# yuanwu2017/llm-d

Measured on AMD Instinct MI355X. Metric: output tok/s per decode GPU + p50 TTFT, Llama-3-70B P/D-disagg on 8×MI355X, higher is better.
Workload: dtype bf16; 1 GPU; model=Llama-3-70B, global_batch=64, seq_len=5000, isl=5000, osl=250, parallelism=dp1, block_size=64, graphs=True, kv_cache_dtype=auto, async_scheduling=True, setup_prompts_landed=63

## Files before the change

### llmd_amd/csrc/ops/bindings.cpp

```cpp
#include <torch/extension.h>
#include <c10/hip/HIPGuard.h>
#include <c10/hip/HIPStream.h>
#include <hip/hip_runtime.h>
#include <pybind11/stl.h>

#include <map>
#include <mutex>
#include <memory>
#include <vector>

extern "C" {
void llmd_rms_norm(void*, int64_t, const void*, int64_t, const void*, int, int, float, hipStream_t);
void llmd_layer_norm(void*, int64_t, void*, int64_t, void*, int64_t, const void*, const void*, int, int, float,
                     hipStream_t);
void llmd_fused_add_rms_norm(void*, int64_t, void*, int64_t, const void*, int, int, float,
                             hipStream_t);
int llmd_qk_rms_norm(void*, int64_t, const void*, const void*, int, int, int, int, float, hipStream_t);
void llmd_rope_cache(void*, int64_t, const int64_t*, const float*, int, int, int, int,
                     const int64_t*, void*, void*, int64_t, int, int, int, int, float, float, hipStream_t);
void llmd_gated_act(void*, int64_t, const void*, int64_t, int, int, int, float, float, hipStream_t);
int llmd_paged_decode(const void*, int64_t, const void*, const void*, int64_t, int, const int*, int,
                      const int*, int, int, int, int, float, int, const float*, int, int, void*,
                      int64_t, float*, float*, int, float, float, const int*, const int*, const int*,
                      const int*, int, int, int, const int*, hipStream_t);
int llmd_paged_prefill(const void*, int64_t, const void*, const void*, int64_t, int, const int*, int,
                       const int*, const int*, const int*, const int*, int, int, int, int, float,
                       int, const float*, void*, int64_t, int, float, float, hipStream_t);
int llmd_prefill_tokens_per_item(int, int, int, int, int);
void llmd_sample(const void*, int64_t, int, int, int, const float*, const int64_t*, int64_t*, float*,
                 float*, int, hipStream_t);
int llmd_sample_splits(int, int);
void llmd_topk_topp_mask(float*, int64_t, int, int, const int*, const float*, const float*,
                         hipStream_t);
void llmd_top_logprobs(const void*, int64_t, int, int, int, const int*, int, int*, float*, hipStream_t);
int llmd_top_logprobs_max();
int llmd_kvx_copy_blocks(void*, const void*, int64_t, int64_t, const int*, int, const int64_t*, int,
                         int64_t, hipStream_t);
int llmd_kvx_copy_blocks2(void*, const void*, int64_t, int64_t, const int*, int, const int64_t*, int, int64_t, int,
                          hipStream_t);
int llmd_kvx_ipc_export(const void*, void*, int64_t*);
int llmd_kvx_ipc_open(const void*, void**);
int llmd_kvx_ipc_close(void*);
int llmd_mla_attention(const void*, int64_t, const void*, int64_t, int, const int*, int, const int*,
                       const int*, int, int, float, int, int, void*, int64_t, float*, float*, int, float,
                       const int*, hipStream_t);
int llmd_mla_rope_cache(const void*, int64_t, void*, int64_t, const void*, int64_t, const void*, int64_t,
                        const int64_t*, const float*, int, int, const int64_t*, void*, int64_t, int, int, float,
                        hipStream_t);
int llmd_lora_bgmv(const void*, int64_t, const void*, const void*, int, int, int, int, const int*, float*, void*,
                   int64_t, hipStream_t);
int llmd_skinny_gemm(const void*, int64_t, const void*, int64_t, int, int, int, int, int, int, void*, int64_t,
                     float*, hipStream_t);
int llmd_dgemm_supported(int, int, int);
int llmd_mgemm(const void*, int64_t, const void*, int64_t, int, int, int, int, int, int, void*, int64_t, float*,
               int*, hipStream_t);
int llmd_mgemm_lds(int, int, int);
int llmd_mgemm_partials(const void*, int64_t, const void*, int64_t, int, int, int, int, int, int, float*, hipStream_t);
int llmd_reduce_rope_cache(const float*, int, int, void*, int64_t, const int64_t*, const float*, int, int, int, int,
                           const int64_t*, void*, void*, int64_t, int, int, int, int, float, float, hipStream_t);
int llmd_mgemm_add_rmsnorm(const void*, int64_t, const void*, int64_t, int, int, int, int, int, int, float*, void*,
                           int64_t, const void*, float, void*, int64_t, hipStream_t);
int llmd_mgemm_silu(const void*, int64_t, const void*, int64_t, int, int, int, int, int, void*, int64_t, hipStream_t);
int llmd_pgemm(const void*, int64_t, const void*, int64_t, void*, int64_t, int, int, int, int, int, void*,
               hipStream_t);
int64_t llmd_pgemm_ws_bytes(int, int, int, int, int);
int llmd_pgemm_fp8(const void*, int64_t, const float*, const void*, int64_t, const float*, void*, int64_t, int, int,
                   int, int, void*, hipStream_t);
int64_t llmd_pgemm_fp8_ws_bytes(int, int, int, int);
int llmd_mgemm_fp8(const void*, int64_t, const float*, const void*, int64_t, const float*, int, int, int, int, int,
                   int, void*, int64_t, float*, int*, hipStream_t);
int llmd_vmm_granularity(int, size_t*);
int llmd_vmm_alloc(int, size_t, int, void**, uint64_t*);
int llmd_vmm_export_fd(uint64_t, int*);
int llmd_vmm_import(const int*, int, size_t, int, void**, uint64_t*);
int llmd_vmm_free(void*, size_t, int, const uint64_t*);
int llmd_kvx_handle_size();
int llmd_kvx_dma_blocks(void*, const void*, int64_t, int64_t, const int*, int, int64_t, hipStream_t);
void llmd_moe_topk(const float*, int, int, int, int, const float*, int, int, int, float, int*, float*,
                   hipStream_t);
void llmd_moe_align(const int*, int, int, int, int*, int*, int*, int, int*, int*, hipStream_t);
int llmd_moe_gemm_tile_m();
void llmd_moe_gemm(const void*, int64_t, int, const int*, const int*, int, const void*, int64_t, int, int,
                   void*, int64_t, int, int, float, float, int, const void*, hipStream_t);
void llmd_moe_combine(const void*, int64_t, const int*, const float*, int, int, int, void*, int64_t,
                      hipStream_t);
int llmd_quant_fp8_rows(const void*, int64_t, void*, int64_t, float*, int, int, hipStream_t);
void llmd_rms_norm_quant(void*, int64_t, float*, const void*, int64_t, void*, int64_t, const void*, int, int, float,
                         hipStream_t);
void llmd_gated_act_quant(void*, int64_t, float*, const void*, int64_t, int, int, int, float, float, hipStream_t);
int llmd_quant_fp8_groups(const void*, int64_t, void*, int64_t, float*, int64_t, int, int, hipStream_t);
int llmd_quant_fp8_groups_padded(const void*, int64_t, void*, int64_t, float*, int64_t, int, int, int, const int*,
                                 hipStream_t);
void llmd_moe_gemm_fp8(const void*, int64_t, const float*, int64_t, int, const int*, const int*, int, const void*,
                       int64_t, const float*, int, int, void*, int64_t, int, int, float, float, int, const void*,
                       hipStream_t);
int llmd_moe_gemm3_fp8(const void*, int64_t, const float*, int64_t, int, const int*, const int*, int, const void*,
                       int64_t, const float*, int, int, void*, int64_t, int, int, float, float, int, const void*,
                       void*, int64_t, float*, int64_t, hipStream_t);
int llmd_moe_gemm3_tile_m();
int llmd_moe_gemm4_bf16(const void*, int64_t, int, const int*, const int*, int, const void*, int64_t, int, int, void*,
                        int64_t, int, int, float, float, int, const void*, int64_t, int, hipStream_t);
int llmd_moe_gemm8_bf16(const void*, int64_t, int, const int*, const int*, const int*, int, const void*, int64_t, int,
                        int, void*, int64_t, int, int, float, float, int, const void*, int64_t, int, hipStream_t);
int llmd_moe_gemm4_fp8(const void*, int64_t, const float*, int64_t, int, const int*, const int*, int, const void*,
                       int64_t, const float*, int, int, void*, int64_t, int, int, float, float, int, const void*,
                       int64_t, int, hipStream_t);
int llmd_moe_gemm8_fp8(const void*, int64_t, const float*, int64_t, int, const int*, const int*, const int*, int,
                       const void*, int64_t, const float*, int, int, void*, int64_t, int, int, float, float, int,
                       const void*, int64_t, int, hipStream_t);
int llmd_moe_gemm3_bf16(const void*, int64_t, int, const int*, const int*, int, const void*, int64_t, int, int, void*,
                        int64_t, int, int, float, float, int, const void*, hipStream_t);
int llmd_symm_alloc(size_t, void**);
int llmd_symm_free(void*);
int64_t llmd_symm_sig_bytes();
int llmd_symm_grid();
int llmd_symm_max_ranks();
int llmd_symm_channels();
int llmd_symm_error(const void*, uint32_t*);
int llmd_symm_clear_error(void*);
int llmd_symm_host_err(int64_t*);
int llmd_symm_all_reduce(const int64_t*, int, int, int, int, int64_t, int64_t, const void*, void*, int64_t,
                         hipStream_t);
int llmd_symm_ep_dispatch(const int64_t*, int, int, int, const int64_t*, const void*, int64_t, const int*,
                          const float*, int, int, int, int, int, int, hipStream_t);
int llmd_symm_ep_combine(const int64_t*, int, int, int, const int64_t*, const void*, int64_t, const int*, int, int,
                         int, int, int, void*, int64_t, hipStream_t);
}

namespace {

std::optional<c10::DeviceIndex> dev_of(const torch::Tensor& t) {
  if (t.is_cuda()) return t.get_device();
  return std::nullopt;
}

hipStream_t cur_stream() { return c10::hip::getCurrentHIPStream().stream(); }

#define CHECK_CUDA(x) TORCH_CHECK((x).is_cuda(), #x " must be a GPU tensor")
#define CHECK_BF16(x) TORCH_CHECK((x).scalar_type() == at::kBFloat16, #x " must be bf16")
#define CHECK_INNER(x) TORCH_CHECK((x).stride(-1) == 1, #x " inner dim must be contiguous")
#define CHECK_DT(x, t) TORCH_CHECK((x).scalar_type() == (t), #x " has wrong dtype")

void rms_norm(torch::Tensor out, torch::Tensor x, torch::Tensor w, double eps) {
  const c10::hip::OptionalHIPGuard device_guard(dev_of(out));
  CHECK_CUDA(x); CHECK_BF16(x); CHECK_BF16(out); CHECK_BF16(w);
  CHECK_INNER(x); CHECK_INNER(out);
  TORCH_CHECK(x.dim() == 2 && out.dim() == 2 && w.is_contiguous(), "rms_norm: 2-D x/out");
  const int d = x.size(1);
  TORCH_CHECK(d % 8 == 0 && w.numel() == d && out.size(1) == d && out.size(0) == x.size(0),
              "rms_norm shape");
  TORCH_CHECK(x.stride(0) % 8 == 0 && out.stride(0) % 8 == 0, "rms_norm: 16-B aligned rows");
  llmd_rms_norm(out.data_ptr(), out.stride(0), x.data_ptr(), x.stride(0), w.data_ptr(), x.size(0), d,
                (float)eps, cur_stream());
}

void qk_rms_norm(torch::Tensor qkv, torch::Tensor qw, torch::Tensor kw, int64_t Hq, int64_t Hkv, double eps) {
  const c10::hip::OptionalHIPGuard device_guard(dev_of(qkv));
  CHECK_CUDA(qkv); CHECK_BF16(qkv); CHECK_BF16(qw); CHECK_BF16(kw);
  CHECK_INNER(qkv);
  TORCH_CHECK(qkv.dim() == 2, "qk_rms_norm: qkv [T, (Hq+2Hkv)*D]");
  const int64_t D = qw.numel();
  TORCH_CHECK(kw.numel() == D && qw.is_contiguous() && kw.is_contiguous(), "qk_rms_norm: weights [D]");
  TORCH_CHECK(D == 64 || D == 128 || D == 256, "qk_rms_norm: head dim 64 / 128 / 256");
  TORCH_CHECK(qkv.size(1) >= (Hq + Hkv) * D, "qk_rms_norm: qkv narrower than (Hq + Hkv) * D");
  const int rc = llmd_qk_rms_norm(qkv.data_ptr(), qkv.stride(0), qw.data_ptr(), kw.data_ptr(), qkv.size(0),
                                  (int)Hq, (int)Hkv, (int)D, (float)eps, cur_stream());
  TORCH_CHECK(rc == 0, "qk_rms_norm: unsupported head dim");
}

void fused_add_rms_norm(torch::Tensor x, torch::Tensor residual, torch::Tensor w, double eps) {
  const c10::hip::OptionalHIPGuard device_guard(dev_of(x));
  CHECK_CUDA(x); CHECK_BF16(x); CHECK_BF16(residual); CHECK_BF16(w);
  CHECK_INNER(x); CHECK_INNER(residual);
  TORCH_CHECK(x.dim() == 2 && residual.sizes() == x.sizes(), "fused_add_rms_norm shape");
  const int d = x.size(1);
  TORCH_CHECK(d % 8 == 0 && w.numel() == d && w.is_contiguous(), "fused_add_rms_norm d");
  TORCH_CHECK(x.stride(0) % 8 == 0 && residual.stride(0) % 8 == 0, "16-B aligned rows");
  llmd_fused_add_rms_norm(x.data_ptr(), x.stride(0), residual.data_ptr(), residual.stride(0),
                          w.data_ptr(), x.size(0), d, (float)eps, cur_stream());
}

void layer_norm(torch::Tensor out, torch::Tensor x, c10::optional<torch::Tensor> residual, torch::Tensor w,
                torch::Tensor b, double eps) {
  const c10::hip::OptionalHIPGuard device_guard(dev_of(x));
  CHECK_CUDA(x); CHECK_BF16(x); CHECK_BF16(out); CHECK_BF16(w); CHECK_BF16(b);
  CHECK_INNER(x); CHECK_INNER(out);
  TORCH_CHECK(x.dim() == 2 && out.sizes() == x.sizes(), "layer_norm: 2-D x/out of one shape");
  const int d = x.size(1);
  TORCH_CHECK(d % 8 == 0 && w.numel() == d && b.numel() == d && w.is_contiguous() && b.is_contiguous(),
              "layer_norm: d % 8 == 0, contiguous w/b of d elements");
  TORCH_CHECK(x.stride(0) % 8 == 0 && out.stride(0) % 8 == 0, "layer_norm: 16-B aligned rows");
  void* rp = nullptr;
  int64_t rs = 0;
  if (residual.has_value()) {
    CHECK_BF16(*residual); CHECK_INNER(*residual);
    TORCH_CHECK(residual->sizes() == x.sizes() && residual->stride(0) % 8 == 0, "layer_norm residual shape");
    rp = residual->data_ptr();
    rs = residual->stride(0);
  }
  llmd_layer_norm(out.data_ptr(), out.stride(0), x.data_ptr(), x.stride(0), rp, rs, w.data_ptr(), b.data_ptr(),
                  x.size(0), d, (float)eps, cur_stream());
}

bool is_fp8_cache(const torch::Tensor& c) {
  TORCH_CHECK(c.is_cuda(), "cache must be a GPU tensor");
  const auto t = c.scalar_type();
  TORCH_CHECK(t == at::kBFloat16 || t == at::kFloat8_e4m3fn, "KV cache must be bf16 or float8_e4m3fn");
  return t == at::kFloat8_e4m3fn;
}

void rope_cache(torch::Tensor qkv, torch::Tensor positions, torch::Tensor cos_sin, int64_t Hq,
                int64_t Hkv, int64_t D, torch::Tensor slots, torch::Tensor k_cache,
                torch::Tensor v_cache, bool neox, double k_scale, double v_scale) {
  const c10::hip::OptionalHIPGuard device_guard(dev_of(qkv));
  CHECK_CUDA(qkv); CHECK_BF16(qkv); CHECK_INNER(qkv);
  CHECK_DT(positions, at::kLong); CHECK_DT(slots, at::kLong); CHECK_DT(cos_sin, at::kFloat);
  TORCH_CHECK(qkv.dim() == 2 && qkv.size(1) >= (Hq + 2 * Hkv) * D, "rope_cache: qkv width");
  const int T = qkv.size(0);
// ... 169 lines not shown
                "mla workspace too small");
  }
  int rc = llmd_mla_attention(q.data_ptr(), q.stride(0), cache.data_ptr(), cache.stride(0), cache.size(1),
                              block_tables.data_ptr<int>(), block_tables.stride(0), row_seq.data_ptr<int>(),
                              row_len.data_ptr<int>(), R, H, (float)scale, split_size, nsplit, out.data_ptr(),
                              out.stride(0), nsplit > 1 ? part_o.data_ptr<float>() : nullptr,
                              nsplit > 1 ? part_ml.data_ptr<float>() : nullptr, f8 ? 1 : 0, (float)kv_scale,
                              sdev, cur_stream());
  TORCH_CHECK(rc == 0, "mla_attention failed: ", rc);
}

void mla_rope_cache(torch::Tensor q, torch::Tensor q_lat, torch::Tensor kv_c, torch::Tensor k_pe,
                    torch::Tensor positions, torch::Tensor cos_sin, int64_t H, torch::Tensor slots,
                    torch::Tensor cache, double kv_scale) {
  const c10::hip::OptionalHIPGuard device_guard(dev_of(q));
  CHECK_CUDA(q); CHECK_BF16(q); CHECK_BF16(q_lat); CHECK_BF16(kv_c); CHECK_BF16(k_pe);
  const bool f8 = is_fp8_cache(cache);
  TORCH_CHECK(kv_scale > 0, "mla_rope: kv_scale must be positive");
  CHECK_INNER(q); CHECK_INNER(q_lat); CHECK_INNER(kv_c); CHECK_INNER(k_pe);
  CHECK_DT(positions, at::kLong); CHECK_DT(slots, at::kLong); CHECK_DT(cos_sin, at::kFloat);
  const int T = q.size(0);
  TORCH_CHECK(q.size(1) >= H * 192 && q_lat.size(0) >= T && q_lat.size(1) >= H * 576, "mla_rope: q widths");
  TORCH_CHECK(kv_c.size(0) >= T && kv_c.size(1) == 512 && k_pe.size(0) >= T && k_pe.size(1) == 64,
              "mla_rope: kv_c [T,512], k_pe [T,64]");
  TORCH_CHECK(kv_c.stride(0) % 8 == 0, "mla_rope: 16-B aligned kv_c rows");
  TORCH_CHECK(positions.numel() >= T && slots.numel() >= T, "mla_rope: positions/slots");
  TORCH_CHECK(cos_sin.dim() == 2 && cos_sin.size(1) == 64 && cos_sin.is_contiguous(), "mla_rope: cos_sin [P,64]");
  TORCH_CHECK(cache.dim() == 3 && cache.size(2) == 576 && cache.stride(1) == 576, "mla_rope: cache [blocks,bs,576]");
  int rc = llmd_mla_rope_cache(q.data_ptr(), q.stride(0), q_lat.data_ptr(), q_lat.stride(0), kv_c.data_ptr(),
                               kv_c.stride(0), k_pe.data_ptr(), k_pe.stride(0), positions.data_ptr<int64_t>(),
                               cos_sin.data_ptr<float>(), T, H, slots.data_ptr<int64_t>(), cache.data_ptr(),
                               cache.stride(0), cache.size(1), f8 ? 1 : 0, (float)(1.0 / kv_scale), cur_stream());
  TORCH_CHECK(rc == 0, "mla_rope_cache failed: ", rc);
}

void lora_bgmv(torch::Tensor y, torch::Tensor x, torch::Tensor A, torch::Tensor B, torch::Tensor slot,
               torch::Tensor h) {
  const c10::hip::OptionalHIPGuard device_guard(dev_of(y));
  CHECK_CUDA(x); CHECK_BF16(x); CHECK_BF16(y); CHECK_BF16(A); CHECK_BF16(B); CHECK_INNER(x); CHECK_INNER(y);
  CHECK_DT(slot, at::kInt); CHECK_DT(h, at::kFloat);
  TORCH_CHECK(A.dim() == 3 && B.dim() == 3 && A.is_contiguous() && B.is_contiguous(), "lora: A [S,R,in], B [S,out,R]");
  const int T = x.size(0), R = A.size(1), in = A.size(2), out = B.size(1);
  TORCH_CHECK(B.size(0) == A.size(0) && B.size(2) == R && R <= 128, "lora: slot/rank mismatch");
  TORCH_CHECK(x.size(1) == in && y.size(0) == T && y.size(1) == out && slot.numel() >= T, "lora: shapes");
  TORCH_CHECK(in % 8 == 0 && in <= 32768 && x.stride(0) % 8 == 0, "lora: in dim");
  TORCH_CHECK(h.numel() >= (int64_t)T * R, "lora: workspace");
  int rc = llmd_lora_bgmv(x.data_ptr(), x.stride(0), A.data_ptr(), B.data_ptr(), T, R, in, out, slot.data_ptr<int>(),
                          h.data_ptr<float>(), y.data_ptr(), y.stride(0), cur_stream());
  TORCH_CHECK(rc == 0, "lora_bgmv failed: ", rc);
}

void skinny_gemm(torch::Tensor y, torch::Tensor x, torch::Tensor w, int64_t rb, int64_t nsplit, int64_t occ,
                 torch::Tensor part) {
  const c10::hip::OptionalHIPGuard device_guard(dev_of(y));
  CHECK_CUDA(x); CHECK_BF16(x); CHECK_BF16(w); CHECK_BF16(y); CHECK_INNER(x); CHECK_INNER(w); CHECK_INNER(y);
  TORCH_CHECK(x.dim() == 2 && w.dim() == 2 && y.dim() == 2, "skinny_gemm: 2-D operands");
  const int M = x.size(0), K = x.size(1), N = w.size(0);
  TORCH_CHECK(M >= 1 && M <= 64 && w.size(1) == K && K % 256 == 0, "skinny_gemm: M <= 64, K % 256 == 0");
  TORCH_CHECK(N % 4 == 0, "skinny_gemm: N % 4 == 0");
  TORCH_CHECK(y.size(0) == M && y.size(1) == N, "skinny_gemm: output shape");
  TORCH_CHECK(x.stride(0) % 8 == 0 && w.stride(0) % 8 == 0 && y.stride(0) % 4 == 0, "skinny_gemm: row alignment");
  TORCH_CHECK(llmd_dgemm_supported(M, (int)rb, (int)occ), "skinny_gemm: no kernel for rb=", rb, " occ=", occ);
  if (nsplit > 1) {
    CHECK_DT(part, at::kFloat);
    TORCH_CHECK(part.numel() >= nsplit * (int64_t)M * N, "skinny_gemm: workspace");
  }
  int rc = llmd_skinny_gemm(x.data_ptr(), x.stride(0), w.data_ptr(), w.stride(0), M, N, K, (int)rb, (int)nsplit,
                            (int)occ, y.data_ptr(), y.stride(0), nsplit > 1 ? part.data_ptr<float>() : nullptr,
                            cur_stream());
  TORCH_CHECK(rc == 0, "skinny_gemm failed: ", rc);
}

extern "C" int llmd_mla_v2_shape(int R, int fp8);
int64_t mla_v2_shape(int64_t R, bool fp8) { return llmd_mla_v2_shape((int)R, fp8 ? 1 : 0); }

bool skinny_supported(int64_t M, int64_t rb, int64_t occ) { return llmd_dgemm_supported((int)M, (int)rb, (int)occ); }

int* mgemm_counters(const torch::Device& d, int64_t tiles) {
  static const bool on = [] {
    const char* e = getenv("LLMD_MGEMM_FIXUP");
    return e && e[0] == '1';
  }();
  if (!on || tiles > 1024) return nullptr;
  static std::mutex mu;
  static std::map<int, torch::Tensor> pools;
  static std::map<int, uint32_t> next;
  std::lock_guard<std::mutex> g(mu);
  auto& t = pools[d.index()];
  if (!t.defined()) {
    hipStreamCaptureStatus cs = hipStreamCaptureStatusNone;
    if (hipStreamIsCapturing(cur_stream(), &cs) != hipSuccess || cs != hipStreamCaptureStatusNone) return nullptr;
    t = torch::zeros({256 * 1024}, torch::dtype(torch::kInt32).device(d));
  }
  const uint32_t i = next[d.index()]++ % 256;
  return t.data_ptr<int>() + (int64_t)i * 1024;
}

void mgemm(torch::Tensor y, torch::Tensor x, torch::Tensor w, int64_t wrb, int64_t nsplit, int64_t stages,
           torch::Tensor part) {
  const c10::hip::OptionalHIPGuard device_guard(dev_of(y));
  CHECK_CUDA(x); CHECK_BF16(x); CHECK_BF16(w); CHECK_BF16(y); CHECK_INNER(x); CHECK_INNER(w); CHECK_INNER(y);
  TORCH_CHECK(x.dim() == 2 && w.dim() == 2 && y.dim() == 2, "mgemm: 2-D operands");
  const int M = x.size(0), K = x.size(1), N = w.size(0);
  TORCH_CHECK(M >= 1 && M <= 256 && w.size(1) == K && K % 64 == 0, "mgemm: M <= 256, K % 64 == 0");
  TORCH_CHECK(N % 4 == 0 && y.size(0) == M && y.size(1) == N, "mgemm: output shape / N % 4");
  TORCH_CHECK(x.stride(0) % 8 == 0 && w.stride(0) % 8 == 0 && y.stride(0) % 4 == 0, "mgemm: row alignment");
  TORCH_CHECK(llmd_mgemm_lds(M, (int)wrb, (int)stages) > 0, "mgemm: no kernel for wrb=", wrb, " stages=", stages);
  if (nsplit > 1) {
    CHECK_DT(part, at::kFloat);
    TORCH_CHECK(part.numel() >= nsplit * (int64_t)M * N, "mgemm: workspace");
  }
  int rc = llmd_mgemm(x.data_ptr(), x.stride(0), w.data_ptr(), w.stride(0), M, N, K, (int)wrb, (int)nsplit,
                      (int)stages, y.data_ptr(), y.stride(0), nsplit > 1 ? part.data_ptr<float>() : nullptr,
                      nsplit > 1 ? mgemm_counters(y.device(), (N + 64 * wrb - 1) / (64 * wrb)) : nullptr,
                      cur_stream());
  TORCH_CHECK(rc == 0, "mgemm failed: ", rc);
}

void mgemm_add_rmsnorm(torch::Tensor out, torch::Tensor x, torch::Tensor w, int64_t wrb, int64_t nsplit,
                       int64_t stages, torch::Tensor part, torch::Tensor residual, torch::Tensor gamma, double eps) {
  const c10::hip::OptionalHIPGuard device_guard(dev_of(out));
  CHECK_CUDA(x); CHECK_BF16(x); CHECK_BF16(w); CHECK_BF16(out); CHECK_BF16(residual); CHECK_BF16(gamma);
  CHECK_INNER(x); CHECK_INNER(w); CHECK_INNER(out); CHECK_INNER(residual); CHECK_DT(part, at::kFloat);
  TORCH_CHECK(x.dim() == 2 && w.dim() == 2 && out.dim() == 2 && residual.dim() == 2, "mgemm_add_rmsnorm: 2-D operands");
  const int M = x.size(0), K = x.size(1), N = w.size(0);
  TORCH_CHECK(M >= 1 && M <= 128 && w.size(1) == K && K % 64 == 0 && N % 8 == 0, "mgemm_add_rmsnorm: shapes");
  TORCH_CHECK(out.size(0) == M && out.size(1) == N && residual.size(0) == M && residual.size(1) == N &&
              gamma.numel() == N, "mgemm_add_rmsnorm: output / residual / gamma shape");
  TORCH_CHECK(nsplit > 1 && part.numel() >= nsplit * (int64_t)M * N, "mgemm_add_rmsnorm: split-K workspace");
  int rc = llmd_mgemm_add_rmsnorm(x.data_ptr(), x.stride(0), w.data_ptr(), w.stride(0), M, N, K, (int)wrb,
                                  (int)nsplit, (int)stages, part.data_ptr<float>(), residual.data_ptr(),
                                  residual.stride(0), gamma.data_ptr(), (float)eps, out.data_ptr(), out.stride(0),
                                  cur_stream());
  TORCH_CHECK(rc == 0, "mgemm_add_rmsnorm failed: ", rc);
}

void pgemm(torch::Tensor y, torch::Tensor x, torch::Tensor w, int64_t epi, int64_t variant, bool split_k) {
  const c10::hip::OptionalHIPGuard device_guard(dev_of(y));
  CHECK_CUDA(x); CHECK_BF16(x); CHECK_BF16(w); CHECK_BF16(y); CHECK_INNER(x); CHECK_INNER(w); CHECK_INNER(y);
  TORCH_CHECK(x.dim() == 2 && w.dim() == 2 && y.dim() == 2, "pgemm: 2-D operands");
  const int64_t M = x.size(0), K = x.size(1), N = w.size(0);
  TORCH_CHECK(w.size(1) == K && K % 64 == 0 && N % 256 == 0, "pgemm: N % 256 == 0, K % 64 == 0");
  TORCH_CHECK(y.size(0) == M && y.size(1) == ((epi == 1 || epi == 3) ? N / 2 : N), "pgemm: output shape");
  TORCH_CHECK(epi != 3 || (variant >= 3 && variant <= 6), "pgemm: epi 3 (SiLU on the [gate; up] weight) needs variant 3-6");
  TORCH_CHECK(x.stride(0) % 8 == 0 && w.stride(0) % 8 == 0 && y.stride(0) % 8 == 0, "pgemm: 16-B row alignment");
  torch::Tensor ws;
  const int64_t wsb = split_k ? llmd_pgemm_ws_bytes((int)M, (int)N, (int)K, (int)epi, (int)variant) : 0;
  if (wsb > 0) ws = torch::empty({wsb / 4}, x.options().dtype(torch::kFloat));
  int rc = llmd_pgemm(x.data_ptr(), x.stride(0), w.data_ptr(), w.stride(0), y.data_ptr(), y.stride(0), (int)M,
                      (int)N, (int)K, (int)epi, (int)variant, wsb > 0 ? ws.data_ptr() : nullptr, cur_stream());
  TORCH_CHECK(rc == 0, "pgemm failed: ", rc);
}

void pgemm_fp8(torch::Tensor y, torch::Tensor xq, torch::Tensor xs, torch::Tensor wq, torch::Tensor ws, int64_t epi,
               bool split_k) {
  const c10::hip::OptionalHIPGuard device_guard(dev_of(y));
  CHECK_CUDA(xq); CHECK_BF16(y); CHECK_INNER(xq); CHECK_INNER(wq); CHECK_INNER(y);
  TORCH_CHECK(xq.scalar_type() == at::kFloat8_e4m3fn && wq.scalar_type() == at::kFloat8_e4m3fn, "pgemm_fp8: e4m3fn");
  TORCH_CHECK(xs.scalar_type() == at::kFloat && ws.scalar_type() == at::kFloat, "pgemm_fp8: fp32 scales");
  TORCH_CHECK(xs.is_contiguous() && ws.is_contiguous(), "pgemm_fp8: contiguous scales");
  TORCH_CHECK(xq.dim() == 2 && wq.dim() == 2 && y.dim() == 2, "pgemm_fp8: 2-D operands");
  const int64_t M = xq.size(0), K = xq.size(1), N = wq.size(0);
  TORCH_CHECK(wq.size(1) == K && K % 128 == 0 && N % 256 == 0, "pgemm_fp8: N % 256 == 0, K % 128 == 0");
  TORCH_CHECK(xs.numel() == M && ws.numel() == N, "pgemm_fp8: per-token / per-channel scales");
  TORCH_CHECK(epi == 0 || epi == 3, "pgemm_fp8: epi 0 or 3");
  TORCH_CHECK(y.size(0) == M && y.size(1) == (epi == 3 ? N / 2 : N), "pgemm_fp8: output shape");
  TORCH_CHECK(xq.stride(0) % 16 == 0 && wq.stride(0) % 16 == 0 && y.stride(0) % 8 == 0, "pgemm_fp8: 16-B rows");
  torch::Tensor wsp;
  const int64_t wsb = split_k ? llmd_pgemm_fp8_ws_bytes((int)M, (int)N, (int)K, (int)epi) : 0;
  if (wsb > 0) wsp = torch::empty({wsb / 4}, xs.options());
  int rc = llmd_pgemm_fp8(xq.data_ptr(), xq.stride(0), xs.data_ptr<float>(), wq.data_ptr(), wq.stride(0),
                          ws.data_ptr<float>(), y.data_ptr(), y.stride(0), (int)M, (int)N, (int)K, (int)epi,
                          wsb > 0 ? wsp.data_ptr() : nullptr, cur_stream());
  TORCH_CHECK(rc == 0, "pgemm_fp8 failed: ", rc);
}

void mgemm_silu(torch::Tensor y, torch::Tensor x, torch::Tensor w, int64_t wrb, int64_t stages) {
  const c10::hip::OptionalHIPGuard device_guard(dev_of(y));
  CHECK_CUDA(x); CHECK_BF16(x); CHECK_BF16(w); CHECK_BF16(y); CHECK_INNER(x); CHECK_INNER(w); CHECK_INNER(y);
  TORCH_CHECK(x.dim() == 2 && w.dim() == 2 && y.dim() == 2, "mgemm_silu: 2-D operands");
  const int M = x.size(0), K = x.size(1), N = w.size(0);
  TORCH_CHECK(M >= 1 && M <= 256 && w.size(1) == K && K % 64 == 0 && N % 8 == 0, "mgemm_silu: shapes");
  TORCH_CHECK(y.size(0) == M && y.size(1) == N / 2, "mgemm_silu: y [M, N / 2]");
  int rc = llmd_mgemm_silu(x.data_ptr(), x.stride(0), w.data_ptr(), w.stride(0), M, N, K, (int)wrb, (int)stages,
                           y.data_ptr(), y.stride(0), cur_stream());
  TORCH_CHECK(rc == 0, "mgemm_silu failed: ", rc);
}

void mgemm_fp8(torch::Tensor y, torch::Tensor xq, torch::Tensor xs, torch::Tensor wq, torch::Tensor ws, int64_t wrb,
               int64_t nsplit, int64_t stages, torch::Tensor part) {
  const c10::hip::OptionalHIPGuard device_guard(dev_of(y));
  CHECK_CUDA(xq); CHECK_BF16(y); CHECK_INNER(xq); CHECK_INNER(wq); CHECK_INNER(y);
  TORCH_CHECK(xq.scalar_type() == at::kFloat8_e4m3fn && wq.scalar_type() == at::kFloat8_e4m3fn, "mgemm_fp8: e4m3fn");
  CHECK_DT(xs, at::kFloat); CHECK_DT(ws, at::kFloat);
  TORCH_CHECK(xq.dim() == 2 && wq.dim() == 2 && y.dim() == 2, "mgemm_fp8: 2-D operands");
  const int M = xq.size(0), K = xq.size(1), N = wq.size(0);
  TORCH_CHECK(M >= 1 && M <= 256 && wq.size(1) == K && K % 128 == 0, "mgemm_fp8: M <= 256, K % 128 == 0");
  TORCH_CHECK(N % 4 == 0 && y.size(0) == M && y.size(1) == N, "mgemm_fp8: output shape / N % 4");
  TORCH_CHECK(xs.is_contiguous() && xs.numel() == M && ws.is_contiguous() && ws.numel() == N, "mgemm_fp8: scales");
  TORCH_CHECK(reinterpret_cast<uintptr_t>(ws.data_ptr()) % 16 == 0, "mgemm_fp8: 16-B aligned weight scales");
  TORCH_CHECK(xq.stride(0) % 16 == 0 && wq.stride(0) % 16 == 0 && y.stride(0) % 4 == 0, "mgemm_fp8: row alignment");
  TORCH_CHECK(llmd_mgemm_lds(M, (int)wrb, (int)stages) > 0, "mgemm_fp8: no kernel for wrb=", wrb, " stages=", stages);
  if (nsplit > 1) {
    CHECK_DT(part, at::kFloat);
    TORCH_CHECK(part.numel() >= nsplit * (int64_t)M * N, "mgemm_fp8: workspace");
  }
  int rc = llmd_mgemm_fp8(xq.data_ptr(), xq.stride(0), xs.data_ptr<float>(), wq.data_ptr(), wq.stride(0),
                          ws.data_ptr<float>(), M, N, K, (int)wrb, (int)nsplit, (int)stages, y.data_ptr(), y.stride(0),
                          nsplit > 1 ? part.data_ptr<float>() : nullptr,
                          nsplit > 1 ? mgemm_counters(y.device(), (N + 64 * wrb - 1) / (64 * wrb)) : nullptr,
                          cur_stream());
  TORCH_CHECK(rc == 0, "mgemm_fp8 failed: ", rc);
}

extern "C" int llmd_kv_dequant_gather(const void*, const void*, int64_t, const int*, int, int, int, void*, void*,
                                      hipStream_t);

void kv_dequant_gather(torch::Tensor k_cache, torch::Tensor v_cache, torch::Tensor block_tables, torch::Tensor kd,
                       torch::Tensor vd) {
  const c10::hip::OptionalHIPGuard device_guard(dev_of(k_cache));
  CHECK_CUDA(k_cache); CHECK_DT(k_cache, at::kFloat8_e4m3fn); CHECK_DT(v_cache, at::kFloat8_e4m3fn);
  CHECK_BF16(kd); CHECK_BF16(vd); CHECK_DT(block_tables, at::kInt);
  TORCH_CHECK(k_cache.dim() == 4 && v_cache.sizes() == k_cache.sizes() && v_cache.stride(0) == k_cache.stride(0),
              "caches [blocks, Hkv, bs, D], same layout");
  const int64_t per = k_cache.size(1) * k_cache.size(2) * k_cache.size(3);
  TORCH_CHECK(k_cache.stride(3) == 1 && k_cache.stride(2) == k_cache.size(3) &&
              k_cache.stride(1) == k_cache.size(2) * k_cache.size(3), "a block's [Hkv, bs, D] contiguous");
  TORCH_CHECK(block_tables.is_contiguous() && kd.is_contiguous() && vd.is_contiguous() &&
              kd.numel() == block_tables.numel() * per && vd.numel() == kd.numel(), "kd / vd [entries, Hkv, bs, D]");
  const int rc = llmd_kv_dequant_gather(k_cache.data_ptr(), v_cache.data_ptr(), k_cache.stride(0),
                                        block_tables.data_ptr<int>(), (int)block_tables.numel(),
                                        (int)k_cache.size(0), (int)per, kd.data_ptr(), vd.data_ptr(), cur_stream());
  TORCH_CHECK(rc == 0, "kv_dequant_gather failed: ", rc);
}

void paged_prefill(torch::Tensor out, torch::Tensor q, torch::Tensor k_cache,
                   torch::Tensor v_cache, torch::Tensor block_tables, torch::Tensor q_start,
                   torch::Tensor q_len, torch::Tensor ctx_len, torch::Tensor items, int64_t Hq,
                   int64_t Hkv, int64_t D, double scale, int64_t window,
                   c10::optional<torch::Tensor> sinks, double k_scale, double v_scale) {
  const c10::hip::OptionalHIPGuard device_guard(dev_of(out));
  CHECK_CUDA(q); CHECK_BF16(q); CHECK_BF16(out); CHECK_INNER(q); CHECK_INNER(out);
  check_cache(k_cache, v_cache, Hkv, D);
  CHECK_DT(block_tables, at::kInt); CHECK_DT(q_start, at::kInt); CHECK_DT(q_len, at::kInt);
  CHECK_DT(ctx_len, at::kInt); CHECK_DT(items, at::kInt);
  TORCH_CHECK(block_tables.dim() == 2 && block_tables.stride(1) == 1, "block_tables 2-D");
  TORCH_CHECK(items.dim() == 2 && items.size(1) == 2 && items.is_contiguous(), "items [n, 2]");
  TORCH_CHECK(Hq % Hkv == 0 && (D == 64 || D == 128), "prefill: heads/D");
  TORCH_CHECK(q.size(1) >= Hq * D && out.size(1) >= Hq * D && out.size(0) >= q.size(0), "widths");
  TORCH_CHECK(q.stride(0) % 8 == 0, "prefill: 16-B aligned q rows");
  const float* sk = nullptr;
  if (sinks.has_value()) {
    CHECK_DT(sinks.value(), at::kFloat);
    TORCH_CHECK(sinks->numel() == Hq, "sinks [Hq]");
    sk = sinks->data_ptr<float>();
  }
  int rc = llmd_paged_prefill(q.data_ptr(), q.stride(0), k_cache.data_ptr(), v_cache.data_ptr(),
                              k_cache.stride(0), k_cache.size(2), block_tables.data_ptr<int>(),
                              block_tables.stride(0), q_start.data_ptr<int>(),
                              q_len.data_ptr<int>(), ctx_len.data_ptr<int>(),
                              items.data_ptr<int>(), items.size(0), Hq, Hkv, D, (float)scale,
                              (int)window, sk, out.data_ptr(), out.stride(0), is_fp8_cache(k_cache) ? 1 : 0,
                              (float)k_scale, (float)v_scale, cur_stream());
  TORCH_CHECK(rc == 0, "paged_prefill: unsupported head dim");
}

void sample(torch::Tensor logits, c10::optional<torch::Tensor> temps,
            c10::optional<torch::Tensor> seeds, torch::Tensor out_ids,
            c10::optional<torch::Tensor> out_logprob) {
  const c10::hip::OptionalHIPGuard device_guard(dev_of(logits));
  CHECK_CUDA(logits); CHECK_INNER(logits);
  TORCH_CHECK(logits.dim() == 2, "logits 2-D");
  const bool bf = logits.scalar_type() == at::kBFloat16;
  TORCH_CHECK(bf || logits.scalar_type() == at::kFloat, "logits bf16/f32");
  const int B = logits.size(0), V = logits.size(1);
  TORCH_CHECK(logits.stride(0) % (bf ? 8 : 4) == 0, "16-B aligned logits rows");
  CHECK_DT(out_ids, at::kLong);
  TORCH_CHECK(out_ids.numel() >= B, "out_ids");
  const float* t = nullptr;
  const int64_t* s = nullptr;
  float* lp = nullptr;
  if (temps.has_value()) { CHECK_DT(temps.value(), at::kFloat); TORCH_CHECK(temps->numel() >= B); t = temps->data_ptr<float>(); }
  if (seeds.has_value()) { CHECK_DT(seeds.value(), at::kLong); TORCH_CHECK(seeds->numel() >= B); s = seeds->data_ptr<int64_t>(); }
  if (out_logprob.has_value()) { CHECK_DT(out_logprob.value(), at::kFloat); lp = out_logprob->data_ptr<float>(); }
  const int nsp = llmd_sample_splits(B, V);
  at::Tensor part;
  if (nsp > 1) part = at::empty({(int64_t)B * nsp * 4}, logits.options().dtype(at::kFloat));
  llmd_sample(logits.data_ptr(), logits.stride(0), B, V, bf ? 1 : 0, t, s,
              out_ids.data_ptr<int64_t>(), lp, nsp > 1 ? part.data_ptr<float>() : nullptr, nsp, cur_stream());
}

void topk_topp_mask(torch::Tensor logits, c10::optional<torch::Tensor> topk,
                    c10::optional<torch::Tensor> topp, c10::optional<torch::Tensor> temps) {
  const c10::hip::OptionalHIPGuard device_guard(dev_of(logits));
  CHECK_CUDA(logits); CHECK_DT(logits, at::kFloat); CHECK_INNER(logits);
  const int B = logits.size(0), V = logits.size(1);
  const int* k = nullptr;
  const float* p = nullptr;
  const float* t = nullptr;
  if (topk.has_value()) { CHECK_DT(topk.value(), at::kInt); TORCH_CHECK(topk->numel() >= B); k = topk->data_ptr<int>(); }
  if (topp.has_value()) { CHECK_DT(topp.value(), at::kFloat); TORCH_CHECK(topp->numel() >= B); p = topp->data_ptr<float>(); }
  if (temps.has_value()) { CHECK_DT(temps.value(), at::kFloat); TORCH_CHECK(temps->numel() >= B); t = temps->data_ptr<float>(); }
  llmd_topk_topp_mask(logits.data_ptr<float>(), logits.stride(0), B, V, k, p, t, cur_stream());
}

void top_logprobs(torch::Tensor logits, torch::Tensor n_per_row, torch::Tensor out_ids, torch::Tensor out_lp) {
// ... 420 lines not shown
  TORCH_CHECK((fused || Y.size(1) >= (mode == 1 ? N / 2 : N)) && N % 2 == 0, "moe_gemm_fp8: Y width");
  const void* bp = nullptr;
  if (bias.has_value()) {
    CHECK_BF16(bias.value());
    TORCH_CHECK(bias->is_contiguous() && bias->numel() == (int64_t)E * N, "bias [E, N]");
    bp = bias->data_ptr();
  }
  void* hqp = nullptr;
  float* hsp = nullptr;
  int64_t hq_stride = 0, hs_stride = 0;
  if (hq.has_value()) {
    TORCH_CHECK(v3 && mode == 1 && hs.has_value(), "fused quant: 256-row tiles, gated activation, hq + hs");
    CHECK_DT(hq.value(), at::kFloat8_e4m3fn); CHECK_INNER(hq.value()); CHECK_DT(hs.value(), at::kFloat);
    TORCH_CHECK(hq->size(0) >= P && hq->size(1) >= ((N / 2 + 127) / 128) * 128 && hq->size(1) % 128 == 0,
                "hq [rows, F rounded up to 128]");
    TORCH_CHECK(hs->dim() == 2 && hs->size(0) >= P && hs->size(1) >= (N + 255) / 256 && hs->stride(1) == 1,
                "hs [rows, F / 128]");
    hqp = hq->data_ptr();
    hsp = hs->data_ptr<float>();
    hq_stride = hq->stride(0);
    hs_stride = hs->stride(0);
  }
  if (v3) {
    TORCH_CHECK(K % 128 == 0 && X.stride(0) % 16 == 0 && W.stride(0) % 16 == 0, "moe_gemm_fp8 (256-row tiles): K");
    const int rc = llmd_moe_gemm3_fp8(X.data_ptr(), X.stride(0), xs.data_ptr<float>(), xs.stride(0), topk,
                                      sorted_ids.data_ptr<int>(), tile_expert.data_ptr<int>(), P / bm, W.data_ptr(),
                                      W.stride(0), ws.data_ptr<float>(), N, K, fused ? nullptr : Y.data_ptr(),
                                      fused ? 0 : Y.stride(0), mode, act, (float)alpha, (float)limit,
                                      a_rows_are_slots ? 1 : 0, bp, hqp, hq_stride, hsp, hs_stride, cur_stream());
    TORCH_CHECK(rc == 0, "moe_gemm3_fp8 failed: ", rc);
    return;
  }
  llmd_moe_gemm_fp8(X.data_ptr(), X.stride(0), xs.data_ptr<float>(), xs.stride(0), topk, sorted_ids.data_ptr<int>(),
                    tile_expert.data_ptr<int>(), P / bm, W.data_ptr(), W.stride(0), ws.data_ptr<float>(), N, K,
                    Y.data_ptr(), Y.stride(0), mode, act, (float)alpha, (float)limit, a_rows_are_slots ? 1 : 0, bp,
                    cur_stream());
}

torch::Tensor symm_alloc(int64_t bytes, int64_t device) {
  const c10::hip::HIPGuard guard((c10::DeviceIndex)device);
  TORCH_CHECK(bytes > llmd_symm_sig_bytes() && bytes % 4096 == 0, "symm_alloc: size");
  void* p = nullptr;
  int rc = llmd_symm_alloc((size_t)bytes, &p);
  TORCH_CHECK(rc == 0, "symm_alloc (hipExtMallocWithFlags uncached) failed: ", rc);
  return torch::from_blob(p, {bytes}, [](void* q) { llmd_symm_free(q); },
                          torch::TensorOptions().dtype(torch::kUInt8).device(torch::kCUDA, (c10::DeviceIndex)device));
}

int64_t symm_error(torch::Tensor heap, bool clear) {
  const c10::hip::OptionalHIPGuard device_guard(dev_of(heap));
  uint32_t e = 0;
  TORCH_CHECK(llmd_symm_error(heap.data_ptr(), &e) == 0, "symm_error: copy failed");
  if (clear) llmd_symm_clear_error(heap.data_ptr());
  return (int64_t)e;
}

int64_t symm_host_err() {
  int64_t p = 0;
  TORCH_CHECK(llmd_symm_host_err(&p) == 0, "symm_host_err: hipHostMalloc failed");
  return p;
}

void check_bases(const std::vector<int64_t>& bases, int64_t rank) {
  TORCH_CHECK((int)bases.size() >= 1 && (int)bases.size() <= llmd_symm_max_ranks(), "symm: 1..8 ranks");
  TORCH_CHECK(rank >= 0 && rank < (int64_t)bases.size(), "symm: rank");
  for (auto b : bases) TORCH_CHECK(b != 0 && b % 256 == 0, "symm: bad peer base");
}

void symm_all_reduce(std::vector<int64_t> bases, int64_t rank, int64_t ch, int64_t mode, int64_t data_off,
                     int64_t slot_bytes, torch::Tensor inp, torch::Tensor out) {
  const c10::hip::OptionalHIPGuard device_guard(dev_of(inp));
  check_bases(bases, rank);
  CHECK_CUDA(inp); CHECK_BF16(inp); CHECK_BF16(out);
  TORCH_CHECK(inp.is_contiguous() && out.is_contiguous() && inp.numel() == out.numel(), "all_reduce: contiguous");
  TORCH_CHECK(inp.numel() % 8 == 0, "all_reduce: numel % 8");
  TORCH_CHECK(data_off >= llmd_symm_sig_bytes() && (mode == 1 || mode == 2), "all_reduce: layout/mode");
  int rc = llmd_symm_all_reduce(bases.data(), (int)bases.size(), (int)rank, (int)ch, (int)mode, data_off, slot_bytes,
                                inp.data_ptr(), out.data_ptr(), inp.numel() / 8, cur_stream());
  TORCH_CHECK(rc == 0, "symm_all_reduce failed: ", rc);
}

void symm_ep_dispatch(std::vector<int64_t> bases, int64_t rank, int64_t ch, std::vector<int64_t> layout,
                      torch::Tensor x, torch::Tensor ids, torch::Tensor w, int64_t R, int64_t E_local, bool fp8) {
  const c10::hip::OptionalHIPGuard device_guard(dev_of(x));
  check_bases(bases, rank);
  CHECK_CUDA(x); CHECK_BF16(x); CHECK_INNER(x); CHECK_DT(ids, at::kInt); CHECK_DT(w, at::kFloat);
  TORCH_CHECK(layout.size() == 7, "ep layout");
  TORCH_CHECK(!fp8 || (layout[5] >= 0 && layout[6] >= 0), "ep_dispatch: heap has no fp8 receive area");
  const int T = x.size(0), d = x.size(1);
  TORCH_CHECK(ids.dim() == 2 && ids.is_contiguous() && w.sizes() == ids.sizes() && w.is_contiguous() &&
                  ids.size(0) == T, "ep_dispatch: ids/w [T, k]");
  const int k = ids.size(1);
  TORCH_CHECK(T <= R && d % 8 == 0 && k <= 64 && x.stride(0) % 8 == 0, "ep_dispatch shape");
  int rc = llmd_symm_ep_dispatch(bases.data(), (int)bases.size(), (int)rank, (int)ch, layout.data(), x.data_ptr(),
                                 x.stride(0), ids.data_ptr<int>(), w.data_ptr<float>(), T, (int)R, d, k, (int)E_local,
                                 (int)fp8, cur_stream());
  TORCH_CHECK(rc == 0, "symm_ep_dispatch failed: ", rc);
}

void symm_ep_combine(std::vector<int64_t> bases, int64_t rank, int64_t ch, std::vector<int64_t> layout,
                     torch::Tensor y, torch::Tensor ids, int64_t R, int64_t E_local, torch::Tensor out) {
  const c10::hip::OptionalHIPGuard device_guard(dev_of(y));
  check_bases(bases, rank);
  CHECK_CUDA(y); CHECK_BF16(y); CHECK_BF16(out); CHECK_INNER(y); CHECK_INNER(out); CHECK_DT(ids, at::kInt);
  TORCH_CHECK(layout.size() == 7, "ep layout");
  const int T = out.size(0), d = out.size(1);
  TORCH_CHECK(ids.dim() == 2 && ids.is_contiguous() && ids.size(0) == T, "ep_combine: ids [T, k]");
  TORCH_CHECK(y.size(0) == (int64_t)bases.size() * R && y.size(1) >= d && d % 8 == 0 && T <= R, "ep_combine shape");
  TORCH_CHECK(y.stride(0) % 8 == 0 && out.stride(0) % 8 == 0, "16-B aligned rows");
  int rc = llmd_symm_ep_combine(bases.data(), (int)bases.size(), (int)rank, (int)ch, layout.data(), y.data_ptr(),
                                y.stride(0), ids.data_ptr<int>(), T, (int)R, d, (int)ids.size(1), (int)E_local,
                                out.data_ptr(), out.stride(0), cur_stream());
  TORCH_CHECK(rc == 0, "symm_ep_combine failed: ", rc);
}

}

PYBIND11_MODULE(TORCH_EXTENSION_NAME, m) {
  m.doc() = "llmd_amd HIP/CDNA4 op library (gfx950)";
  m.def("rms_norm", &rms_norm);
  m.def("fused_add_rms_norm", &fused_add_rms_norm);
  m.def("qk_rms_norm", &qk_rms_norm, "Qwen3 per-head q/k RMSNorm in place in the fused QKV output");
  m.def("layer_norm", &layer_norm);
  m.def("rope_cache", &rope_cache);
  m.def("gated_act", &gated_act);
  m.def("paged_decode", &paged_decode);
  m.def("paged_prefill", &paged_prefill);
  m.def("kv_dequant_gather", &kv_dequant_gather);
  m.def("moe_gemm8_mxfp4", &moe_gemm8_mxfp4);
  m.def("prefill_tokens_per_item", [](int64_t Hq, int64_t Hkv, int64_t D, int64_t bs, bool fp8) {
    return llmd_prefill_tokens_per_item((int)Hq, (int)Hkv, (int)D, (int)bs, fp8 ? 1 : 0);
  });
  m.def("sample", &sample);
  m.def("topk_topp_mask", &topk_topp_mask);
  m.def("top_logprobs", &top_logprobs);
  m.def("top_logprobs_max", &llmd_top_logprobs_max);
  m.def("kvx_copy_blocks", &kvx_copy_blocks);
  m.def("kvx_dma_blocks", &kvx_dma_blocks);
  m.def("kvx_ipc_export", &kvx_ipc_export);
  m.def("kvx_ipc_open", &kvx_ipc_open);
  m.def("kvx_ipc_close", &kvx_ipc_close);
  m.def("mla_attention", &mla_attention);
  m.def("mla_v2_shape", &mla_v2_shape, "H=128 MLA kernel shape: 10 * waves + head blocks per wave");
  m.def("skinny_gemm", &skinny_gemm);
  m.def("skinny_supported", &skinny_supported);
  m.def("mgemm", &mgemm);
  m.def("mgemm_partials", &mgemm_partials, "split-K partials of the medium-M GEMM (no reduce); returns nsplit");
  m.def("reduce_rope_cache", &reduce_rope_cache, "QKV split-K reduce + RoPE + paged cache write");
  m.def("mgemm_add_rmsnorm", &mgemm_add_rmsnorm, "decode o / down projection with residual-add + RMSNorm in its split-K reduce");
  m.def("pgemm_fp8", &pgemm_fp8, "prefill fp8 W8A8 GEMM (256x256 LDS-DMA tiles on 16x16x128 f8f6f4 MFMA), "
        "per-token x per-channel scales, optional fused SiLU-and-mul");
  m.def("pgemm", &pgemm, "prefill bf16 GEMM (256x256 LDS-DMA MFMA tiles), optional fused SiLU-and-mul",
        py::arg("y"), py::arg("x"), py::arg("w"), py::arg("epi"), py::arg("variant"), py::arg("split_k") = true);
  m.def("mgemm_fp8", &mgemm_fp8);
  m.def("mgemm_lds", [](int64_t M, int64_t wrb, int64_t stages) { return llmd_mgemm_lds((int)M, (int)wrb, (int)stages); });
  m.def("lora_bgmv", &lora_bgmv);
  m.def("mla_rope_cache", &mla_rope_cache);
  m.def("vmm_granularity", &vmm_granularity);
  m.def("vmm_pool", &vmm_pool);
  m.def("vmm_import", &vmm_import);
  m.def("vmm_release", &vmm_release);
  m.def("moe_topk", &moe_topk);
  m.def("moe_align", &moe_align, py::arg("ids"), py::arg("E"), py::arg("sorted_ids"), py::arg("tile_expert"),
        py::arg("expert_offsets"), py::arg("total_p"), py::arg("inv"), py::arg("tile_m") = 0);
  m.def("moe_gemm", &moe_gemm, py::arg("X"), py::arg("topk"), py::arg("sorted_ids"), py::arg("tile_expert"),
        py::arg("W"), py::arg("Y"), py::arg("mode"), py::arg("act"), py::arg("alpha"), py::arg("limit"),
        py::arg("a_rows_are_slots"), py::arg("bias"), py::arg("tile_m") = 0);
  m.def("moe_combine", &moe_combine);
  m.def("moe_tile_m", &llmd_moe_gemm_tile_m);
  m.def("quant_fp8_rows", &quant_fp8_rows);
  m.def("quant_fp8_groups", &quant_fp8_groups);
  m.def("quant_fp8_groups_padded", &quant_fp8_groups_padded, py::arg("x"), py::arg("q"), py::arg("scale"),
        py::arg("row_limit") = py::none());
  m.def("rms_norm_quant", &rms_norm_quant);
  m.def("gated_act_quant", &gated_act_quant);
  m.def("moe_gemm_fp8", &moe_gemm_fp8, py::arg("X"), py::arg("xs"), py::arg("topk"), py::arg("sorted_ids"),
        py::arg("tile_expert"), py::arg("W"), py::arg("ws"), py::arg("Y"), py::arg("mode"), py::arg("act"),
        py::arg("alpha"), py::arg("limit"), py::arg("a_rows_are_slots"), py::arg("bias"), py::arg("tile_m") = 0,
        py::arg("hq") = py::none(), py::arg("hs") = py::none());
  m.def("moe_tile_m_prefill", &llmd_moe_gemm3_tile_m);
  m.def("symm_alloc", &symm_alloc);
  m.def("moe_gemm4", &moe_gemm4, py::arg("X"), py::arg("topk"), py::arg("sorted_ids"), py::arg("tile_expert"),
        py::arg("W"), py::arg("Y"), py::arg("mode"), py::arg("act"), py::arg("alpha"), py::arg("limit"),
        py::arg("a_rows_are_slots"), py::arg("bias"), py::arg("tile_m") = 256, py::arg("version") = 4,
        py::arg("total") = py::none());
  m.def("mgemm_silu", &mgemm_silu);
  m.def("moe_gemm4_fp8", &moe_gemm4_fp8, py::arg("X"), py::arg("xs"), py::arg("topk"), py::arg("sorted_ids"),
        py::arg("tile_expert"), py::arg("W"), py::arg("ws"), py::arg("Y"), py::arg("mode"), py::arg("act"),
        py::arg("alpha"), py::arg("limit"), py::arg("a_rows_are_slots"), py::arg("bias"), py::arg("tile_m") = 256,
        py::arg("version") = 4, py::arg("total") = py::none());
  m.def("symm_error", &symm_error);
  m.def("symm_host_err", &symm_host_err);
  m.def("symm_sig_bytes", &llmd_symm_sig_bytes);
  m.def("symm_grid", &llmd_symm_grid);
  m.def("symm_channels", &llmd_symm_channels);
  m.def("symm_all_reduce", &symm_all_reduce);
  m.def("symm_ep_dispatch", &symm_ep_dispatch, py::arg("bases"), py::arg("rank"), py::arg("ch"), py::arg("layout"),
        py::arg("x"), py::arg("ids"), py::arg("w"), py::arg("R"), py::arg("E_local"), py::arg("fp8") = false);
  m.def("symm_ep_combine", &symm_ep_combine);
}
```

### llmd_amd/csrc/ops/pgemm.hip

```cpp
#include <algorithm>
#include <type_traits>

#include "llmd_common.h"

using namespace llmd;

namespace {

constexpr int BM = 256, BN = 256, BK = 64, NT = 512;
constexpr int HALF = 16384;
constexpr int BUF = 4 * HALF;
constexpr int LDS_BYTES = 2 * BUF;
constexpr int GROUP_M = 8;

enum { EPI_NONE = 0, EPI_SILU = 1, EPI_F32 = 2, EPI_SILU_STD = 3 };

__device__ __forceinline__ void dma16(const void* src, char* lds) {
  __builtin_amdgcn_global_load_lds((const void __attribute__((address_space(1)))*)src,
                                   (void __attribute__((address_space(3)))*)lds, 16, 0, 0);
}

__device__ __forceinline__ void wait_vm(int n) {
  switch (n) {
    case 0: asm volatile("s_waitcnt vmcnt(0)" ::: "memory"); break;
    case 2: asm volatile("s_waitcnt vmcnt(2)" ::: "memory"); break;
    case 4: asm volatile("s_waitcnt vmcnt(4)" ::: "memory"); break;
    case 6: asm volatile("s_waitcnt vmcnt(6)" ::: "memory"); break;
    case 8: asm volatile("s_waitcnt vmcnt(8)" ::: "memory"); break;
    default: asm volatile("s_waitcnt vmcnt(10)" ::: "memory"); break;
  }
}

__device__ __forceinline__ void bar() {
  __builtin_amdgcn_sched_barrier(0);
  __builtin_amdgcn_s_barrier();
  __builtin_amdgcn_sched_barrier(0);
}

__device__ __forceinline__ void tile_mn(int L, int tiles_m, int tiles_n, int& tm, int& tn) {
  const int per_group = GROUP_M * tiles_n;
  const int g = L / per_group, first_m = g * GROUP_M;
  const int gm = min(tiles_m - first_m, GROUP_M);
  tm = first_m + (L % per_group) % gm;
  tn = (L % per_group) / gm;
}

template <int EPI>
__global__ __launch_bounds__(NT, 1) void pgemm_kernel(const uint16_t* __restrict__ A, int64_t lda,
                                                      const uint16_t* __restrict__ W, int64_t ldw,
                                                      uint16_t* __restrict__ C, int64_t ldc, int M, int N, int K,
                                                      int tile0, int nsplit, float* __restrict__ ws) {
  __shared__ __attribute__((aligned(1024))) char lds[LDS_BYTES];
  const int tiles_m = (M + BM - 1) / BM, tiles_n = N / BN;
  const int b = xcd_remap(blockIdx.x, gridDim.x);
  const int tail = gridDim.x / nsplit;
  const int t_local = b % tail, split = b / tail;
  const int nk_all = K / BK;
  const int chunk = (nk_all + nsplit - 1) / nsplit;
  const int kbeg = split * chunk;
  const int nk = min(chunk, nk_all - kbeg);
  int tm, tn;
  tile_mn(tile0 + t_local, tiles_m, tiles_n, tm, tn);
  const int m0 = tm * BM, n0 = tn * BN;
  A += (int64_t)kbeg * BK;
  W += (int64_t)kbeg * BK;

  const int tid = threadIdx.x, w = tid >> 6, lane = tid & 63;
  const int wr = w >> 2, wc = w & 3;

  uint32_t aoff[2][2], woff[2][2];
#pragma unroll
  for (int h = 0; h < 2; ++h)
#pragma unroll
    for (int j = 0; j < 2; ++j) {
      const int i = 8 * (2 * w + j) + (lane >> 3);
      const int c = (lane & 7) ^ (i & 7);
      const int ar = min(m0 + (i >> 6) * 128 + h * 64 + (i & 63), M - 1);
      const int wn = n0 + (i >> 5) * 64 + h * 32 + (i & 31);
      aoff[h][j] = (uint32_t)(ar * lda + c * 8);
      woff[h][j] = (uint32_t)(wn * ldw + c * 8);
    }
  auto issue = [&](int seq) {
    const int kt = seq >> 2, kind = seq & 3;
    char* dst = lds + (kt & 1) * BUF + (2 * w) * 1024;
    const int k0 = kt * BK;
    if (kind == 0 || kind == 3) {
      const int h = kind == 0 ? 0 : 1;
      dst += h * HALF;
      dma16(A + aoff[h][0] + k0, dst);
      dma16(A + aoff[h][1] + k0, dst + 1024);
    } else {
      const int h = kind - 1;
      dst += 2 * HALF + h * HALF;
      dma16(W + woff[h][0] + k0, dst);
      dma16(W + woff[h][1] + k0, dst + 1024);
    }
  };
  const int nseq = 4 * nk;
  int issued = 0;
  auto issue_upto = [&](int seq) {
    if (seq < nseq) {
      issue(seq);
      issued = seq + 1;
    }
  };
  auto wait_seq = [&](int seq) { wait_vm(min(5, max(0, issued - seq - 1)) * 2); };

  const int fr = lane & 15, fq = lane >> 4;
  int a_rd[4][2], w_rd[2][2];
#pragma unroll
  for (int mi = 0; mi < 4; ++mi)
#pragma unroll
    for (int s = 0; s < 2; ++s) {
      const int i = wr * 64 + mi * 16 + fr;
      a_rd[mi][s] = i * 128 + (((4 * s + fq) ^ (i & 7)) * 16);
    }
#pragma unroll
  for (int ni = 0; ni < 2; ++ni)
#pragma unroll
    for (int s = 0; s < 2; ++s) {
      const int i = wc * 32 + ni * 16 + fr;
      w_rd[ni][s] = i * 128 + (((4 * s + fq) ^ (i & 7)) * 16);
    }

  f32x4_t acc[2][2][4][2];
#pragma unroll
  for (int a = 0; a < 2; ++a)
#pragma unroll
    for (int b = 0; b < 2; ++b)
#pragma unroll
      for (int c = 0; c < 4; ++c)
#pragma unroll
        for (int d = 0; d < 2; ++d) acc[a][b][c][d] = f32x4_t{0.f, 0.f, 0.f, 0.f};

  s16x8_t afr[4][2], wfr[2][2][2];
  auto read_a = [&](const char* hb) {
#pragma unroll
    for (int mi = 0; mi < 4; ++mi)
#pragma unroll
      for (int s = 0; s < 2; ++s) afr[mi][s] = *reinterpret_cast<const s16x8_t*>(hb + a_rd[mi][s]);
  };
  auto read_w = [&](const char* hb, int qn) {
#pragma unroll
    for (int ni = 0; ni < 2; ++ni)
#pragma unroll
      for (int s = 0; s < 2; ++s) wfr[qn][ni][s] = *reinterpret_cast<const s16x8_t*>(hb + w_rd[ni][s]);
  };
  auto mfma_q = [&](int qm, int qn) {
    __builtin_amdgcn_s_setprio(1);
#pragma unroll
    for (int s = 0; s < 2; ++s)
#pragma unroll
      for (int mi = 0; mi < 4; ++mi)
#pragma unroll
        for (int ni = 0; ni < 2; ++ni)
          acc[qm][qn][mi][ni] =
              __builtin_amdgcn_mfma_f32_16x16x32_bf16(wfr[qn][ni][s], afr[mi][s], acc[qm][qn][mi][ni], 0, 0, 0);
    __builtin_amdgcn_s_setprio(0);
  };
  auto seg_end = [&]() {
    __builtin_amdgcn_s_waitcnt(0xC07F);
    bar();
  };

#pragma unroll
  for (int s = 0; s < 7; ++s) issue_upto(s);
  wait_seq(1);
  bar();
// ... 320 lines not shown
  W += (int64_t)kbeg * BK;

  const int tid = threadIdx.x, w = tid >> 6, lane = tid & 63;
  const int wr = w >> 1, wc = w & 1;

  const int srow = tid >> 3, sc = tid & 7;
  uint32_t aoff[8];
#pragma unroll
  for (int i = 0; i < 8; ++i) aoff[i] = (uint32_t)(min(m0 + 32 * i + srow, M - 1) * lda + sc * 8);
  const uint32_t woff0 = (uint32_t)((n0 + srow) * ldw + sc * 8);
  const uint32_t wstep = (uint32_t)(32 * ldw);
  const int st_off = srow * 128 + swz5(srow, sc) * 16;

  const int fr = lane & 15, fq = lane >> 4;
  const int rd0 = fr * 128 + swz5(fr, fq) * 16, rd1 = fr * 128 + swz5(fr, 4 + fq) * 16;
  const int a_rd = (wr * 128) * 128, w_rd = OPB5 + (wc * 128) * 128;

  f32x4_t acc[8][8];
#pragma unroll
  for (int i = 0; i < 8; ++i)
#pragma unroll
    for (int j = 0; j < 8; ++j) acc[i][j] = f32x4_t{0.f, 0.f, 0.f, 0.f};
  s16x8_t fa0[8], fw0[8], fa1[8], fw1[8];
  u32x4_t ga[8], gw[8];

  auto gload = [&](int kt, int i) {
    const int k0 = min(kt, nk - 1) * BK;
    ga[i] = *reinterpret_cast<const u32x4_t*>(A + aoff[i] + k0);
    gw[i] = *reinterpret_cast<const u32x4_t*>(W + woff0 + i * wstep + k0);
  };
  auto swrite = [&](char* buf, int i) {
    *reinterpret_cast<u32x4_t*>(buf + i * 4096 + st_off) = ga[i];
    *reinterpret_cast<u32x4_t*>(buf + OPB5 + i * 4096 + st_off) = gw[i];
  };

#pragma unroll
  for (int i = 0; i < 8; ++i) gload(0, i);
#pragma unroll
  for (int i = 0; i < 8; ++i) swrite(lds, i);
#pragma unroll
  for (int i = 0; i < 8; ++i) gload(1, i);
  __builtin_amdgcn_s_waitcnt(0xC07F);
  bar();
#pragma unroll
  for (int i = 0; i < 8; ++i) {
    fw0[i] = *reinterpret_cast<const s16x8_t*>(lds + w_rd + i * 2048 + rd0);
    fa0[i] = *reinterpret_cast<const s16x8_t*>(lds + a_rd + i * 2048 + rd0);
  }
  __builtin_amdgcn_sched_barrier(0);
  asm volatile("s_nop 4" ::: "memory");
  __builtin_amdgcn_sched_barrier(0);

#define PG5_ROW(fa, fw, i, SIDE)                                                       \
  {                                                                                    \
    _Pragma("unroll") for (int j = 0; j < 8; ++j) mfma16_acc(acc[i][j], fw[j], fa[i]); \
    SIDE;                                                                              \
    __builtin_amdgcn_sched_barrier(0);                                                 \
  }
  for (int kt = 0; kt < nk; ++kt) {
    char* cur = lds + (kt & 1) * BUF5;
    char* nxt = lds + ((kt & 1) ^ 1) * BUF5;
#pragma unroll
    for (int i = 0; i < 8; ++i) {
      PG5_ROW(fa0, fw0, i, {
        if (i < 4) {
          fw1[2 * i] = *reinterpret_cast<const s16x8_t*>(cur + w_rd + (2 * i) * 2048 + rd1);
          fw1[2 * i + 1] = *reinterpret_cast<const s16x8_t*>(cur + w_rd + (2 * i + 1) * 2048 + rd1);
        } else {
          fa1[2 * i - 8] = *reinterpret_cast<const s16x8_t*>(cur + a_rd + (2 * i - 8) * 2048 + rd1);
          fa1[2 * i - 7] = *reinterpret_cast<const s16x8_t*>(cur + a_rd + (2 * i - 7) * 2048 + rd1);
        }
        swrite(nxt, i);
      });
    }
    __builtin_amdgcn_s_waitcnt(0xC07F);
    bar();
#pragma unroll
    for (int i = 0; i < 8; ++i) {
      PG5_ROW(fa1, fw1, i, {
        if (i < 4) {
          fw0[2 * i] = *reinterpret_cast<const s16x8_t*>(nxt + w_rd + (2 * i) * 2048 + rd0);
          fw0[2 * i + 1] = *reinterpret_cast<const s16x8_t*>(nxt + w_rd + (2 * i + 1) * 2048 + rd0);
        } else {
          fa0[2 * i - 8] = *reinterpret_cast<const s16x8_t*>(nxt + a_rd + (2 * i - 8) * 2048 + rd0);
          fa0[2 * i - 7] = *reinterpret_cast<const s16x8_t*>(nxt + a_rd + (2 * i - 7) * 2048 + rd0);
        }
        gload(kt + 2, i);
      });
    }
  }
#undef PG5_ROW
  mfma_drain();
  __builtin_amdgcn_sched_barrier(0);
  asm volatile("s_waitcnt vmcnt(0) lgkmcnt(0)" ::: "memory");
  if constexpr (EPI == EPI_F32) {
    float* wt = ws + ((int64_t)split * tail + t_local) * (BM * BN);
#pragma unroll
    for (int i = 0; i < 8; ++i)
#pragma unroll
      for (int j = 0; j < 8; ++j) {
        const int row = wr * 128 + 16 * i + fr, col = wc * 128 + 16 * j + 4 * fq;
        *reinterpret_cast<f32x4_t*>(wt + row * BN + col) = acc[i][j];
      }
    return;
  }
  __syncthreads();
  char* img = lds + w * 32768;
#pragma unroll
  for (int i = 0; i < 8; ++i)
#pragma unroll
    for (int j = 0; j < 8; ++j) {
      const int row = 16 * i + fr, col = 16 * j + 4 * fq;
      const f32x4_t v = acc[i][j];
      u32x2_t p;
      p[0] = (uint32_t)f2bf(v[0]) | ((uint32_t)f2bf(v[1]) << 16);
      p[1] = (uint32_t)f2bf(v[2]) | ((uint32_t)f2bf(v[3]) << 16);
      *reinterpret_cast<u32x2_t*>(img + row * 256 + (((col >> 3) ^ (row & 15)) * 16) + (col & 7) * 2) = p;
    }
  __syncthreads();
  if constexpr (EPI == EPI_NONE) {
#pragma unroll 4
    for (int it = 0; it < 32; ++it) {
      const int row = it * 4 + (lane >> 4), c = lane & 15;
      const int m = m0 + wr * 128 + row;
      const u32x4_t v = *reinterpret_cast<const u32x4_t*>(img + row * 256 + ((c ^ (row & 15)) * 16));
      if (m < M) *reinterpret_cast<u32x4_t*>(C + (int64_t)m * ldc + n0 + wc * 128 + c * 8) = v;
    }
  } else {
    const char* gimg = lds + (wr * 2) * 32768;
    const char* uimg = gimg + 32768;
#pragma unroll 4
    for (int it = 0; it < 16; ++it) {
      const int row = wc * 64 + it * 4 + (lane >> 4), c = lane & 15;
      const int m = m0 + wr * 128 + row;
      const int off = row * 256 + ((c ^ (row & 15)) * 16);
      float gf[8], uf[8], of[8];
      unpack8(*reinterpret_cast<const u32x4_t*>(gimg + off), gf);
      unpack8(*reinterpret_cast<const u32x4_t*>(uimg + off), uf);
#pragma unroll
      for (int e = 0; e < 8; ++e) of[e] = gf[e] / (1.f + __expf(-gf[e])) * uf[e];
      if (m < M) *reinterpret_cast<u32x4_t*>(C + (int64_t)m * ldc + n0 / 2 + c * 8) = pack8(of);
    }
  }
}

constexpr int NT6 = 256;
constexpr int OPB6 = BM * BK * 2;
constexpr int BUF6 = 2 * OPB6;

template <int EPI, int RB6 = 37, int AUX6 = 0>
__global__ __launch_bounds__(NT6, 1) void pgemm6_kernel(const uint16_t* __restrict__ A, int64_t lda,
                                                        const uint16_t* __restrict__ W, int64_t ldw,
                                                        uint16_t* __restrict__ C, int64_t ldc, int M, int N, int K,
                                                        int tile0, int nsplit, float* __restrict__ ws) {
  __shared__ __attribute__((aligned(1024))) char lds[2 * BUF6];
  const int tiles_m = (M + BM - 1) / BM, tiles_n = N / BN;
  const int b = xcd_remap(blockIdx.x, gridDim.x);
  const int tail = gridDim.x / nsplit;
  const int t_local = b % tail, split = b / tail;
  const int nk_all = K / BK;
  const int chunk = (nk_all + nsplit - 1) / nsplit;
  const int kbeg = split * chunk;
  const int nk = min(chunk, nk_all - kbeg);
  int tm, tn;
  tile_mn(tile0 + t_local, tiles_m, tiles_n, tm, tn);
  const int m0 = tm * BM, n0 = tn * BN;

  const int tid = threadIdx.x, lane = tid & 63;
  const int w = __builtin_amdgcn_readfirstlane(tid >> 6);
  const int wr = w >> 1, wc = w & 1;

  const __amdgpu_buffer_rsrc_t ra =
      __builtin_amdgcn_make_buffer_rsrc((void*)(A + (int64_t)kbeg * BK), 0, 0x7fffffff, 0x00020000);
  const __amdgpu_buffer_rsrc_t rw =
      __builtin_amdgcn_make_buffer_rsrc((void*)(W + (int64_t)kbeg * BK), 0, 0x7fffffff, 0x00020000);
  uint32_t va[8], vw[8];
#pragma unroll
  for (int j = 0; j < 8; ++j) {
    const int row = 64 * w + 8 * j + (lane >> 3);
    const int c = (lane & 7) ^ ((row >> 1) & 7);
    va[j] = m0 + row < M ? (uint32_t)(((m0 + row) * lda + c * 8) * 2) : 0x80000000u;
    const int wrow = EPI == EPI_SILU_STD ? (row < 128 ? 0 : N / 2 - 128) + tn * 128 + row : n0 + row;
    vw[j] = (uint32_t)((wrow * ldw + c * 8) * 2);
  }
  auto dma = [&](int kt, int j, bool wop) {
    const uint32_t so = (uint32_t)(min(kt, nk - 1) * BK * 2);
    char* dst = lds + (kt & 1) * BUF6 + (wop ? OPB6 : 0) + (8 * w + j) * 1024;
    __builtin_amdgcn_raw_ptr_buffer_load_lds(wop ? rw : ra, (__attribute__((address_space(3))) void*)dst, 16,
                                             wop ? vw[j] : va[j], so, 0, AUX6);
  };

  const int fr = lane & 15, fq = lane >> 4;
  const int rd0 = fr * 128 + ((fq ^ ((fr >> 1) & 7)) * 16);
  const int rd1 = fr * 128 + (((4 + fq) ^ ((fr >> 1) & 7)) * 16);
  const int a_rd = (wr * 128) * 128, w_rd = OPB6 + (wc * 128) * 128;

  f32x4_t acc[8][8];
#pragma unroll
  for (int i = 0; i < 8; ++i)
#pragma unroll
    for (int j = 0; j < 8; ++j) acc[i][j] = f32x4_t{0.f, 0.f, 0.f, 0.f};
  s16x8_t fa0[8], fw0[8], fa1[8], fw1[8];

#pragma unroll
  for (int j = 0; j < 8; ++j) dma(0, j, false);
#pragma unroll
  for (int j = 0; j < 8; ++j) dma(0, j, true);
#pragma unroll
  for (int j = 0; j < 8; ++j) dma(1, j, false);
#pragma unroll
  for (int j = 0; j < 8; ++j) dma(1, j, true);
  asm volatile("s_waitcnt vmcnt(16)" ::: "memory");
  bar();
  fa0[0] = *reinterpret_cast<const s16x8_t*>(lds + a_rd + rd0);
  __builtin_amdgcn_sched_barrier(0);
#pragma unroll
  for (int i = 0; i < 8; ++i) {
    fw0[i] = *reinterpret_cast<const s16x8_t*>(lds + w_rd + i * 2048 + rd0);
    __builtin_amdgcn_sched_barrier(0);
  }
#pragma unroll
  for (int i = 1; i < 8; ++i) {
    fa0[i] = *reinterpret_cast<const s16x8_t*>(lds + a_rd + i * 2048 + rd0);
    __builtin_amdgcn_sched_barrier(0);
  }
  __builtin_amdgcn_s_waitcnt(0xC07F);
  __builtin_amdgcn_sched_barrier(0);
  asm volatile("s_nop 4" ::: "memory");
  __builtin_amdgcn_sched_barrier(0);

  for (int kt = 0; kt < nk; ++kt) {
    const char* cur = lds + (kt & 1) * BUF6;
    const char* nxt = lds + ((kt & 1) ^ 1) * BUF6;
#pragma unroll
    for (int t = 0; t < 64; ++t) {
      const int i = t >> 3, j = t & 7;
      if (t <= 8) __builtin_amdgcn_s_waitcnt(0xC07F | (14 << 8));
      mfma16_acc(acc[i][j], fw0[j], fa0[i]);
      if (t == 0) {
        fa1[0] = *reinterpret_cast<const s16x8_t*>(cur + a_rd + rd1);
      } else if (t < 9) {
        fw1[t - 1] = *reinterpret_cast<const s16x8_t*>(cur + w_rd + (t - 1) * 2048 + rd1);
      } else if (t < 16) {
        fa1[t - 8] = *reinterpret_cast<const s16x8_t*>(cur + a_rd + (t - 8) * 2048 + rd1);
      } else if (t == 40) {
        __builtin_amdgcn_s_waitcnt(0xC07F);
        bar();
      } else if (t > 40 && (t - 41) % 3 == 0) {
        dma(kt + 2, (t - 41) / 3, false);
      }
      __builtin_amdgcn_sched_barrier(0);
    }
#pragma unroll
    for (int t = 0; t < 64; ++t) {
      const int i = t >> 3, j = t & 7;
      mfma16_acc(acc[i][j], fw1[j], fa1[i]);
      if (t < 36 && t % 5 == 0) {
        dma(kt + 2, t / 5, true);
      } else if (t == RB6 - 1) {
        asm volatile("s_waitcnt vmcnt(16)" ::: "memory");
        bar();
      } else if (t == RB6) {
        fa0[0] = *reinterpret_cast<const s16x8_t*>(nxt + a_rd + rd0);
      } else if (t > RB6 && t < RB6 + 9) {
        fw0[t - RB6 - 1] = *reinterpret_cast<const s16x8_t*>(nxt + w_rd + (t - RB6 - 1) * 2048 + rd0);
      } else if (t >= RB6 + 9 && t < RB6 + 16) {
        fa0[t - RB6 - 8] = *reinterpret_cast<const s16x8_t*>(nxt + a_rd + (t - RB6 - 8) * 2048 + rd0);
      }
      __builtin_amdgcn_sched_barrier(0);
    }
  }
  mfma_drain();
  __builtin_amdgcn_sched_barrier(0);
  asm volatile("s_waitcnt vmcnt(0) lgkmcnt(0)" ::: "memory");
  if constexpr (EPI == EPI_F32) {
    float* wt = ws + ((int64_t)split * tail + t_local) * (BM * BN);
#pragma unroll
    for (int i = 0; i < 8; ++i)
#pragma unroll
      for (int j = 0; j < 8; ++j) {
        const int row = wr * 128 + 16 * i + fr, col = wc * 128 + 16 * j + 4 * fq;
        *reinterpret_cast<f32x4_t*>(wt + row * BN + col) = acc[i][j];
      }
    return;
  }
  __syncthreads();
  char* img = lds + w * 32768;
#pragma unroll
  for (int i = 0; i < 8; ++i)
#pragma unroll
    for (int j = 0; j < 8; ++j) {
      const int row = 16 * i + fr, col = 16 * j + 4 * fq;
      const f32x4_t v = acc[i][j];
      u32x2_t p;
      p[0] = (uint32_t)f2bf(v[0]) | ((uint32_t)f2bf(v[1]) << 16);
      p[1] = (uint32_t)f2bf(v[2]) | ((uint32_t)f2bf(v[3]) << 16);
      *reinterpret_cast<u32x2_t*>(img + row * 256 + (((col >> 3) ^ (row & 15)) * 16) + (col & 7) * 2) = p;
    }
  __syncthreads();
  if constexpr (EPI == EPI_NONE) {
#pragma unroll 4
    for (int it = 0; it < 32; ++it) {
      const int row = it * 4 + (lane >> 4), c = lane & 15;
      const int m = m0 + wr * 128 + row;
      const u32x4_t v = *reinterpret_cast<const u32x4_t*>(img + row * 256 + ((c ^ (row & 15)) * 16));
      if (m < M) *reinterpret_cast<u32x4_t*>(C + (int64_t)m * ldc + n0 + wc * 128 + c * 8) = v;
    }
  } else {
    const char* gimg = lds + (wr * 2) * 32768;
    const char* uimg = gimg + 32768;
#pragma unroll 4
    for (int it = 0; it < 16; ++it) {
      const int row = wc * 64 + it * 4 + (lane >> 4), c = lane & 15;
      const int m = m0 + wr * 128 + row;
      const int off = row * 256 + ((c ^ (row & 15)) * 16);
      float gf[8], uf[8], of[8];
      unpack8(*reinterpret_cast<const u32x4_t*>(gimg + off), gf);
      unpack8(*reinterpret_cast<const u32x4_t*>(uimg + off), uf);
#pragma unroll
      for (int e = 0; e < 8; ++e) of[e] = gf[e] / (1.f + __expf(-gf[e])) * uf[e];
      if (m < M) *reinterpret_cast<u32x4_t*>(C + (int64_t)m * ldc + n0 / 2 + c * 8) = pack8(of);
    }
  }
}

template <int EPI>
__global__ __launch_bounds__(NT6, 1) void pgemm7_kernel(const uint16_t* __restrict__ A, int64_t lda,
                                                        const uint16_t* __restrict__ W, int64_t ldw,
                                                        uint16_t* __restrict__ C, int64_t ldc, int M, int N, int K,
                                                        int ntiles) {
  constexpr int RB = 37;
  __shared__ __attribute__((aligned(1024))) char lds[2 * BUF6];
  const int tiles_m = (M + BM - 1) / BM, tiles_n = N / BN;
  const int P = gridDim.x;
  const int b = xcd_remap(blockIdx.x, P);
  const int nt = (ntiles - b + P - 1) / P;
  const int nk = K / BK;
  const int S = nt * nk;

  const int tid = threadIdx.x, lane = tid & 63;
  const int w = __builtin_amdgcn_readfirstlane(tid >> 6);
  const int wr = w >> 1, wc = w & 1;
  const __amdgpu_buffer_rsrc_t ra = __builtin_amdgcn_make_buffer_rsrc((void*)A, 0, 0x7fffffff, 0x00020000);
  const __amdgpu_buffer_rsrc_t rw = __builtin_amdgcn_make_buffer_rsrc((void*)W, 0, 0x7fffffff, 0x00020000);

  uint32_t va[8], vw[8];
  auto set_dma_tile = [&](int r) {
    int tm, tn;
    tile_mn(b + min(r, nt - 1) * P, tiles_m, tiles_n, tm, tn);
#pragma unroll
    for (int j = 0; j < 8; ++j) {
      const int row = 64 * w + 8 * j + (lane >> 3);
      const int c = (lane & 7) ^ ((row >> 1) & 7);
      va[j] = tm * BM + row < M ? (uint32_t)(((tm * BM + row) * lda + c * 8) * 2) : 0x80000000u;
      const int wrow = EPI == EPI_SILU_STD ? (row < 128 ? 0 : N / 2 - 128) + tn * 128 + row : tn * BN + row;
      vw[j] = (uint32_t)((wrow * ldw + c * 8) * 2);
    }
  };
  auto dma = [&](int g, int kt_of_g, int j, bool wop) {
    const uint32_t so = (uint32_t)(kt_of_g * BK * 2);
    char* dst = lds + (g & 1) * BUF6 + (wop ? OPB6 : 0) + (8 * w + j) * 1024;
    __builtin_amdgcn_raw_ptr_buffer_load_lds(wop ? rw : ra, (__attribute__((address_space(3))) void*)dst, 16,
                                             wop ? vw[j] : va[j], so, 0, 0);
  };

  const int fr = lane & 15, fq = lane >> 4;
  const int rd0 = fr * 128 + ((fq ^ ((fr >> 1) & 7)) * 16);
  const int rd1 = fr * 128 + (((4 + fq) ^ ((fr >> 1) & 7)) * 16);
  const int a_rd = (wr * 128) * 128;
  auto w_off = [&](int j) {
    return OPB6 + (EPI == EPI_SILU_STD ? (j < 4 ? wc * 64 + 16 * j : 128 + wc * 64 + 16 * (j - 4))
                                       : wc * 128 + 16 * j) * 128;
  };

  f32x4_t acc[8][8];
#pragma unroll
  for (int i = 0; i < 8; ++i)
#pragma unroll
    for (int j = 0; j < 8; ++j) acc[i][j] = f32x4_t{0.f, 0.f, 0.f, 0.f};
  s16x8_t fa0[8], fw0[8], fa1[8], fw1[8];

  set_dma_tile(0);
#pragma unroll
  for (int j = 0; j < 8; ++j) dma(0, 0, j, false);
#pragma unroll
  for (int j = 0; j < 8; ++j) dma(0, 0, j, true);
  if (nk == 1) set_dma_tile(1);
  const int kt1 = nk == 1 ? 0 : 1;
#pragma unroll
  for (int j = 0; j < 8; ++j) dma(1, kt1, j, false);
#pragma unroll
  for (int j = 0; j < 8; ++j) dma(1, kt1, j, true);
  asm volatile("s_waitcnt vmcnt(16)" ::: "memory");
  bar();
  fa0[0] = *reinterpret_cast<const s16x8_t*>(lds + a_rd + rd0);
  __builtin_amdgcn_sched_barrier(0);
#pragma unroll
  for (int i = 0; i < 8; ++i) {
    fw0[i] = *reinterpret_cast<const s16x8_t*>(lds + w_off(i) + rd0);
    __builtin_amdgcn_sched_barrier(0);
  }
#pragma unroll
  for (int i = 1; i < 8; ++i) {
    fa0[i] = *reinterpret_cast<const s16x8_t*>(lds + a_rd + i * 2048 + rd0);
    __builtin_amdgcn_sched_barrier(0);
  }
  __builtin_amdgcn_s_waitcnt(0xC07F);
  __builtin_amdgcn_sched_barrier(0);
  asm volatile("s_nop 4" ::: "memory");
  __builtin_amdgcn_sched_barrier(0);

  for (int r = 0; r < nt; ++r) {
  for (int kt = 0; kt < nk; ++kt) {
    const int g = r * nk + kt;
    const char* cur = lds + (g & 1) * BUF6;
    const char* nxt = lds + ((g & 1) ^ 1) * BUF6;
    int kt2 = kt + 2;
    if (nk == 1) {
      kt2 = 0;
      set_dma_tile(r + 2);
    } else if (kt2 >= nk) {
      kt2 -= nk;
      if (kt2 == 0) set_dma_tile(r + 1);
    }
    if (g + 2 >= S) kt2 = nk - 1;
#pragma unroll
    for (int t = 0; t < 64; ++t) {
      const int i = t >> 3, j = t & 7;
      if (t <= 8) __builtin_amdgcn_s_waitcnt(0xC07F | (14 << 8));
      mfma16_acc(acc[i][j], fw0[j], fa0[i]);
      if (t == 0) {
        fa1[0] = *reinterpret_cast<const s16x8_t*>(cur + a_rd + rd1);
      } else if (t < 9) {
        fw1[t - 1] = *reinterpret_cast<const s16x8_t*>(cur + w_off(t - 1) + rd1);
      } else if (t < 16) {
        fa1[t - 8] = *reinterpret_cast<const s16x8_t*>(cur + a_rd + (t - 8) * 2048 + rd1);
      } else if (t == 40) {
        __builtin_amdgcn_s_waitcnt(0xC07F);
        bar();
      } else if (t > 40 && (t - 41) % 3 == 0) {
        dma(g + 2, kt2, (t - 41) / 3, false);
      }
      __builtin_amdgcn_sched_barrier(0);
    }
#pragma unroll
    for (int t = 0; t < 64; ++t) {
      const int i = t >> 3, j = t & 7;
      mfma16_acc(acc[i][j], fw1[j], fa1[i]);
      if (t < 36 && t % 5 == 0) {
        dma(g + 2, kt2, t / 5, true);
      } else if (t == RB - 1) {
        asm volatile("s_waitcnt vmcnt(16)" ::: "memory");
        bar();
      } else if (t == RB) {
        fa0[0] = *reinterpret_cast<const s16x8_t*>(nxt + a_rd + rd0);
      } else if (t > RB && t < RB + 9) {
        fw0[t - RB - 1] = *reinterpret_cast<const s16x8_t*>(nxt + w_off(t - RB - 1) + rd0);
      } else if (t >= RB + 9 && t < RB + 16) {
        fa0[t - RB - 8] = *reinterpret_cast<const s16x8_t*>(nxt + a_rd + (t - RB - 8) * 2048 + rd0);
      }
      __builtin_amdgcn_sched_barrier(0);
    }
  }
    {
      int tm, tn;
      tile_mn(b + r * P, tiles_m, tiles_n, tm, tn);
      mfma_drain();
      __builtin_amdgcn_sched_barrier(0);
      const int mrow = tm * BM + wr * 128 + fr;
      if constexpr (EPI == EPI_NONE) {
        uint16_t* cb = C + (int64_t)tn * BN + wc * 128 + 4 * fq;
#pragma unroll
        for (int i = 0; i < 8; ++i) {
          const int m = mrow + 16 * i;
#pragma unroll
          for (int j = 0; j < 8; ++j) {
            const f32x4_t v = acc[i][j];
            u32x2_t p;
            p[0] = (uint32_t)f2bf(v[0]) | ((uint32_t)f2bf(v[1]) << 16);
            p[1] = (uint32_t)f2bf(v[2]) | ((uint32_t)f2bf(v[3]) << 16);
            if (m < M) *reinterpret_cast<u32x2_t*>(cb + (int64_t)m * ldc + 16 * j) = p;
          }
        }
      } else {
        uint16_t* cb = C + (int64_t)tn * 128 + wc * 64 + 4 * fq;
#pragma unroll
        for (int i = 0; i < 8; ++i) {
          const int m = mrow + 16 * i;
#pragma unroll
          for (int j = 0; j < 4; ++j) {
            const f32x4_t gv = acc[i][j], uv = acc[i][j + 4];
            float o[4];
#pragma unroll
            for (int e = 0; e < 4; ++e) o[e] = gv[e] / (1.f + __expf(-gv[e])) * uv[e];
            u32x2_t p;
            p[0] = (uint32_t)f2bf(o[0]) | ((uint32_t)f2bf(o[1]) << 16);
            p[1] = (uint32_t)f2bf(o[2]) | ((uint32_t)f2bf(o[3]) << 16);
            if (m < M) *reinterpret_cast<u32x2_t*>(cb + (int64_t)m * ldc + 16 * j) = p;
          }
        }
      }
#pragma unroll
      for (int i = 0; i < 8; ++i)
#pragma unroll
        for (int j = 0; j < 8; ++j) acc[i][j] = f32x4_t{0.f, 0.f, 0.f, 0.f};
      __builtin_amdgcn_sched_barrier(0);
      asm volatile("s_nop 4" ::: "memory");
      __builtin_amdgcn_sched_barrier(0);
    }
  }
  asm volatile("s_waitcnt vmcnt(0) lgkmcnt(0)" ::: "memory");
}

__global__ __launch_bounds__(256) void pgemm_splitk_reduce(const float* __restrict__ ws, int nsplit, int tail,
                                                           int tile0, uint16_t* __restrict__ C, int64_t ldc, int M,
                                                           int N) {
  const int t = blockIdx.x / (BM / 8), rblk = blockIdx.x % (BM / 8);
  int tm, tn;
  tile_mn(tile0 + t, (M + BM - 1) / BM, N / BN, tm, tn);
  const int row = rblk * 8 + (threadIdx.x >> 5), col = (threadIdx.x & 31) * 8;
  const int m = tm * BM + row;
  if (m >= M) return;
  float f[8] = {0, 0, 0, 0, 0, 0, 0, 0};
  for (int s = 0; s < nsplit; ++s) {
    const float* p = ws + ((int64_t)s * tail + t) * (BM * BN) + row * BN + col;
    const f32x4_t a = *reinterpret_cast<const f32x4_t*>(p), b = *reinterpret_cast<const f32x4_t*>(p + 4);
#pragma unroll
    for (int e = 0; e < 4; ++e) {
      f[e] += a[e];
      f[4 + e] += b[e];
    }
  }
  *reinterpret_cast<u32x4_t*>(C + (int64_t)m * ldc + tn * BN + col) = pack8(f);
}

constexpr int PG_CUS = 256;

__host__ inline void pgemm_plan(int M, int N, int K, int epi, int& full, int& tail, int& nsplit) {
  const int ntiles = ((M + BM - 1) / BM) * (N / BN), nk = K / BK;
  full = ntiles;
  tail = 0;
  nsplit = 1;
  const int t = ntiles % PG_CUS;
  if (epi != EPI_NONE || t == 0 || 2 * t > PG_CUS || nk < 32) return;
  int s = PG_CUS / t;
  s = std::min(s, nk / 8);
  if (s < 2) return;
  full = ntiles - t;
  tail = t;
  nsplit = s;
}

}

extern "C" int64_t llmd_pgemm_ws_bytes(int M, int N, int K, int epi, int variant) {
  if (M <= 0 || N % BN || K % BK) return 0;
  int full, tail, nsplit;
  pgemm_plan(M, N, K, epi, full, tail, nsplit);
  return nsplit > 1 ? (int64_t)nsplit * tail * BM * BN * 4 : 0;
}

extern "C" int llmd_pgemm(const void* A, int64_t lda, const void* W, int64_t ldw, void* C, int64_t ldc, int M, int N,
                          int K, int epi, int variant, void* ws, hipStream_t st) {
  if (M <= 0) return 0;
  if (N % BN || K % BK || lda % 8 || ldw % 8 || ldc % 8) return -1;
  if (epi == EPI_SILU_STD && (variant < 3 || variant > 6)) return -3;
  if ((int64_t)(M - 1) * lda + K > 0x7fffffffLL || (int64_t)(N - 1) * ldw + K > 0x7fffffffLL) return -2;
  const int ntiles = ((M + BM - 1) / BM) * (N / BN);
  if (variant == 6) {
    if (((int64_t)(M - 1) * lda + K) * 2 > 0x7fffffffLL || ((int64_t)(N - 1) * ldw + K) * 2 > 0x7fffffffLL) return -2;
    int full = ntiles, tail = 0, nsplit = 1;
    if (ws != nullptr) pgemm_plan(M, N, K, epi == EPI_SILU_STD ? EPI_SILU : epi, full, tail, nsplit);
    const auto* a = (const uint16_t*)A;
    const auto* w = (const uint16_t*)W;
    auto* c = (uint16_t*)C;
    const int P = std::min(full, PG_CUS);
    if (epi == EPI_SILU_STD)
      hipLaunchKernelGGL(pgemm7_kernel<EPI_SILU_STD>, dim3(P), dim3(NT6), 0, st, a, lda, w, ldw, c, ldc, M, N, K, full);
    else if (epi == EPI_NONE && full > 0)
      hipLaunchKernelGGL(pgemm7_kernel<EPI_NONE>, dim3(P), dim3(NT6), 0, st, a, lda, w, ldw, c, ldc, M, N, K, full);
    else if (epi != EPI_NONE)
      return -3;
    if (nsplit > 1) {
      hipLaunchKernelGGL((pgemm6_kernel<EPI_F32, 37, 0>), dim3(tail * nsplit), dim3(NT6), 0, st, a, lda, w, ldw, c, ldc,
                         M, N, K, full, nsplit, (float*)ws);
      hipLaunchKernelGGL(pgemm_splitk_reduce, dim3(tail * (BM / 8)), dim3(256), 0, st, (const float*)ws, nsplit,
                         tail, full, c, ldc, M, N);
    }
    return (int)hipGetLastError();
  }
  if (variant >= 3 && variant <= 5) {
    if (((int64_t)(M - 1) * lda + K) * 2 > 0x7fffffffLL || ((int64_t)(N - 1) * ldw + K) * 2 > 0x7fffffffLL) return -2;
    int full = ntiles, tail = 0, nsplit = 1;
    if (ws != nullptr) pgemm_plan(M, N, K, epi, full, tail, nsplit);
    const auto* a = (const uint16_t*)A;
    const auto* w = (const uint16_t*)W;
    auto* c = (uint16_t*)C;
    auto launch = [&](auto k_silu, auto k_std, auto k_none, auto k_f32) {
      if (epi == EPI_SILU)
        hipLaunchKernelGGL(k_silu, dim3(full), dim3(NT6), 0, st, a, lda, w, ldw, c, ldc, M, N, K, 0, 1, nullptr);
      else if (epi == EPI_SILU_STD)
        hipLaunchKernelGGL(k_std, dim3(full), dim3(NT6), 0, st, a, lda, w, ldw, c, ldc, M, N, K, 0, 1, nullptr);
      else if (full > 0)
        hipLaunchKernelGGL(k_none, dim3(full), dim3(NT6), 0, st, a, lda, w, ldw, c, ldc, M, N, K, 0, 1, nullptr);
      if (nsplit > 1) {
        hipLaunchKernelGGL(k_f32, dim3(tail * nsplit), dim3(NT6), 0, st, a, lda, w, ldw, c, ldc, M, N, K, full,
                           nsplit, (float*)ws);
        hipLaunchKernelGGL(pgemm_splitk_reduce, dim3(tail * (BM / 8)), dim3(256), 0, st, (const float*)ws, nsplit,
                           tail, full, c, ldc, M, N);
      }
    };
    if (variant == 3)
      launch(pgemm6_kernel<EPI_SILU, 37, 0>, pgemm6_kernel<EPI_SILU_STD, 37, 0>, pgemm6_kernel<EPI_NONE, 37, 0>,
             pgemm6_kernel<EPI_F32, 37, 0>);
    else if (variant == 4)
      launch(pgemm6_kernel<EPI_SILU, 37, 16>, pgemm6_kernel<EPI_SILU_STD, 37, 16>, pgemm6_kernel<EPI_NONE, 37, 16>,
             pgemm6_kernel<EPI_F32, 37, 16>);
    else
      launch(pgemm6_kernel<EPI_SILU, 44, 0>, pgemm6_kernel<EPI_SILU_STD, 44, 0>, pgemm6_kernel<EPI_NONE, 44, 0>,
             pgemm6_kernel<EPI_F32, 44, 0>);
    return (int)hipGetLastError();
  }
  if (variant == 2) {
    int full = ntiles, tail = 0, nsplit = 1;
    if (ws != nullptr) pgemm_plan(M, N, K, epi, full, tail, nsplit);
    const auto* a = (const uint16_t*)A;
    const auto* w = (const uint16_t*)W;
    auto* c = (uint16_t*)C;
    if (epi == EPI_SILU)
      hipLaunchKernelGGL(pgemm5_kernel<EPI_SILU>, dim3(full), dim3(NT5), 0, st, a, lda, w, ldw, c, ldc, M, N, K, 0, 1,
                         nullptr);
    else if (full > 0)
      hipLaunchKernelGGL(pgemm5_kernel<EPI_NONE>, dim3(full), dim3(NT5), 0, st, a, lda, w, ldw, c, ldc, M, N, K, 0, 1,
                         nullptr);
    if (nsplit > 1) {
      hipLaunchKernelGGL(pgemm5_kernel<EPI_F32>, dim3(tail * nsplit), dim3(NT5), 0, st, a, lda, w, ldw, c, ldc, M, N,
                         K, full, nsplit, (float*)ws);
      hipLaunchKernelGGL(pgemm_splitk_reduce, dim3(tail * (BM / 8)), dim3(256), 0, st, (const float*)ws, nsplit,
                         tail, full, c, ldc, M, N);
    }
    return (int)hipGetLastError();
  }
  if (variant == 1) {
    int full = ntiles, tail = 0, nsplit = 1;
    if (ws != nullptr) pgemm_plan(M, N, K, epi, full, tail, nsplit);
    const auto* a = (const uint16_t*)A;
    const auto* w = (const uint16_t*)W;
    auto* c = (uint16_t*)C;
    if (epi == EPI_SILU)
      hipLaunchKernelGGL(pgemm4_kernel<EPI_SILU>, dim3(full), dim3(NT4), 0, st, a, lda, w, ldw, c, ldc, M, N, K, 0, 1,
                         nullptr);
    else if (full > 0)
      hipLaunchKernelGGL(pgemm4_kernel<EPI_NONE>, dim3(full), dim3(NT4), 0, st, a, lda, w, ldw, c, ldc, M, N, K, 0, 1,
                         nullptr);
    if (nsplit > 1) {
      hipLaunchKernelGGL(pgemm4_kernel<EPI_F32>, dim3(tail * nsplit), dim3(NT4), 0, st, a, lda, w, ldw, c, ldc, M, N,
                         K, full, nsplit, (float*)ws);
      hipLaunchKernelGGL(pgemm_splitk_reduce, dim3(tail * (BM / 8)), dim3(256), 0, st, (const float*)ws, nsplit,
                         tail, full, c, ldc, M, N);
    }
    return (int)hipGetLastError();
  }
  int full = ntiles, tail = 0, nsplit = 1;
  if (ws != nullptr) pgemm_plan(M, N, K, epi, full, tail, nsplit);
  const auto* a = (const uint16_t*)A;
  const auto* w = (const uint16_t*)W;
  auto* c = (uint16_t*)C;
  if (epi == EPI_SILU)
    hipLaunchKernelGGL(pgemm_kernel<EPI_SILU>, dim3(full), dim3(NT), 0, st, a, lda, w, ldw, c, ldc, M, N, K, 0, 1,
                       nullptr);
  else if (full > 0)
    hipLaunchKernelGGL(pgemm_kernel<EPI_NONE>, dim3(full), dim3(NT), 0, st, a, lda, w, ldw, c, ldc, M, N, K, 0, 1,
                       nullptr);
  if (nsplit > 1) {
    hipLaunchKernelGGL(pgemm_kernel<EPI_F32>, dim3(tail * nsplit), dim3(NT), 0, st, a, lda, w, ldw, c, ldc, M, N, K,
                       full, nsplit, (float*)ws);
    hipLaunchKernelGGL(pgemm_splitk_reduce, dim3(tail * (BM / 8)), dim3(256), 0, st, (const float*)ws, nsplit, tail,
                       full, c, ldc, M, N);
  }
  return (int)hipGetLastError();
}
```

### llmd_amd/models/layers.py

```python
from __future__ import annotations

import contextlib
import math
import os
from typing import Optional

import torch
import torch.nn.functional as F

from llmd_amd import ops
from llmd_amd.engine.attn_meta import AttnMeta
from llmd_amd.parallel.comm import tp_all_gather, tp_all_reduce
from llmd_amd.parallel.state import get_state


def _init_weight(t: torch.Tensor, std: float, gen: Optional[torch.Generator] = None):
    with torch.no_grad():
        if t.is_cuda:
            t.normal_(0.0, std, generator=gen)
        else:
            t.copy_(torch.randn(t.shape, generator=gen) * std)
    return t


# ... 52 lines not shown
        return ops.moe_experts_mxfp4(x, ids, w, mod.w1, mod.w1_scale, mod.w2, mod.w2_scale, act, alpha, limit,
                                     b1=b1, b2=b2)
    if mod.w1.dtype == torch.float8_e4m3fn:
        return ops.moe_experts_fp8(x, ids, w, mod.w1, mod.w1_scale, mod.w2, mod.w2_scale, act, alpha, limit,
                                   b1=b1, b2=b2)
    if isinstance(x, ops.Fp8Rows):
        x = x.dequant()
    return ops.moe_experts(x, ids, w, mod.w1, mod.w2, act, alpha, limit, b1=b1, b2=b2)


class ColumnLinear(torch.nn.Module):

    def __init__(self, in_f: int, out_f: int, bias=False, device=None, dtype=torch.bfloat16,
                 shard=True, std=0.02):
        super().__init__()
        tp = get_state().tp_size if shard else 1
        assert out_f % tp == 0, (out_f, tp)
        self.in_f, self.out_f = in_f, out_f // tp
        self.weight = torch.nn.Parameter(_init_weight(torch.empty(self.out_f, in_f, device=device, dtype=dtype), std),
                                         requires_grad=False)
        self.bias = torch.nn.Parameter(torch.zeros(self.out_f, device=device, dtype=dtype),
                                       requires_grad=False) if bias else None

    lora = None

    def forward(self, x):
        y = _linear(self, x, self.bias)
        if self.lora is not None:
            self.lora.apply(y, x)
        return y


class RowLinear(torch.nn.Module):

    def __init__(self, in_f: int, out_f: int, bias=False, device=None, dtype=torch.bfloat16,
                 reduce=True, std=0.02):
        super().__init__()
        tp = get_state().tp_size
        assert in_f % tp == 0
        self.in_f, self.out_f, self.reduce = in_f // tp, out_f, reduce
        self.weight = torch.nn.Parameter(_init_weight(torch.empty(out_f, self.in_f, device=device, dtype=dtype), std),
                                         requires_grad=False)
        self.bias = torch.nn.Parameter(torch.zeros(out_f, device=device, dtype=dtype),
                                       requires_grad=False) if bias else None

    lora = None

    def forward(self, x):
        fold = self.bias is not None and self.lora is None and (not self.reduce or get_state().tp_size == 1)
        y = _linear(self, x, self.bias if fold else None)
        if self.lora is not None:
            self.lora.apply(y, x)
        if self.reduce:
            y = tp_all_reduce(y)
        if self.bias is not None and not fold:
            y = y + self.bias
        return y


class RMSNorm(torch.nn.Module):
    def __init__(self, d: int, eps: float, device=None, dtype=torch.bfloat16):
        super().__init__()
        self.eps = eps
        self.weight = torch.nn.Parameter(torch.ones(d, device=device, dtype=dtype), requires_grad=False)

    def forward(self, x, residual: Optional[torch.Tensor] = None, quant: bool = False):
        if quant:
            q = ops.rms_norm_quant(x, self.weight, self.eps, residual)
            return q if residual is None else (q, residual)
        if residual is None:
            return ops.rms_norm(x, self.weight, self.eps)
        ops.fused_add_rms_norm(x, residual, self.weight, self.eps)
        return x, residual


class VocabEmbedding(torch.nn.Module):

    def __init__(self, vocab: int, d: int, device=None, dtype=torch.bfloat16):
        super().__init__()
        st = get_state()
        self.tp, self.rank = st.tp_size, st.tp_rank
        self.vocab = vocab
        self.per = math.ceil(math.ceil(vocab / self.tp) / 64) * 64
        self.lo = self.rank * self.per
        self.weight = torch.nn.Parameter(_init_weight(torch.empty(self.per, d, device=device, dtype=dtype), 0.02),
                                         requires_grad=False)

    def forward(self, ids):
        if self.tp == 1:
            return F.embedding(ids, self.weight)
        local = ids - self.lo
        mask = (local < 0) | (local >= self.per)
        out = F.embedding(local.clamp(0, self.per - 1), self.weight)
        out.masked_fill_(mask[:, None], 0)
        return tp_all_reduce(out)


class LMHead(torch.nn.Module):
    def __init__(self, vocab: int, d: int, device=None, dtype=torch.bfloat16, tied: Optional[VocabEmbedding] = None):
        super().__init__()
        st = get_state()
        self.tp = st.tp_size
        self.vocab = vocab
        self.per = math.ceil(math.ceil(vocab / self.tp) / 64) * 64
        if tied is not None:
            self.weight = tied.weight
        else:
            self.weight = torch.nn.Parameter(_init_weight(torch.empty(self.per, d, device=device, dtype=dtype), 0.02),
                                             requires_grad=False)

    def forward(self, h):
        logits = F.linear(h, self.weight)
        if self.tp > 1:
            logits = tp_all_gather(logits, -1)
        return logits[:, : self.vocab]


_ATTN_OVERLAP = os.environ.get("LLMD_ATTN_OVERLAP", "1") == "1"
_SIDE_STREAMS: dict = {}


def _overlap_stream(t: torch.Tensor):
    if not (_ATTN_OVERLAP and t.is_cuda) or torch.cuda.is_current_stream_capturing():
        return None
    s = _SIDE_STREAMS.get(t.device.index)
    if s is None:
        s = _SIDE_STREAMS[t.device.index] = torch.cuda.Stream(device=t.device)
    return s


class PagedAttention(torch.nn.Module):

    def __init__(self, layer_idx: int, num_heads: int, num_kv_heads: int, head_dim: int,
                 rope_cos_sin: torch.Tensor, window: int = 0, sinks: bool = False, neox: bool = True,
                 device=None):
        super().__init__()
        tp = get_state().tp_size
        assert num_heads % tp == 0
        self.layer_idx = layer_idx
        self.Hq = num_heads // tp
        self.Hkv = max(1, num_kv_heads // tp)
        self.D = head_dim
        self.scale = head_dim ** -0.5
        self.window = window
        self.neox = neox
        self.cos_sin = rope_cos_sin
        self.sinks = torch.nn.Parameter(torch.zeros(self.Hq, device=device, dtype=torch.float32),
                                        requires_grad=False) if sinks else None
        self.k_cache: Optional[torch.Tensor] = None
        self.v_cache: Optional[torch.Tensor] = None
        self.k_scale = 1.0
        self.v_scale = 1.0

    def forward(self, qkv: torch.Tensor, meta: AttnMeta, parts=None) -> torch.Tensor:
        T = qkv.shape[0]
        Hq, Hkv, D = self.Hq, self.Hkv, self.D
        if self.window and meta.swa is not None:
            meta = meta.swa
        if parts is not None:
            ops.reduce_rope_cache(parts[0], parts[1], qkv, meta.positions, self.cos_sin, Hq, Hkv, D,
                                  meta.slot_mapping, self.k_cache, self.v_cache, self.neox, self.k_scale,
                                  self.v_scale)
        else:
            ops.rope_cache(qkv, meta.positions, self.cos_sin, Hq, Hkv, D, meta.slot_mapping,
                           self.k_cache, self.v_cache, self.neox, self.k_scale, self.v_scale)
        out = torch.empty(T, Hq * D, dtype=qkv.dtype, device=qkv.device)
        nd = meta.num_decode
        side = _overlap_stream(qkv) if nd and meta.num_prefill_tokens else None
        if nd:
            if side is not None:
                side.wait_stream(torch.cuda.current_stream(qkv.device))
            with torch.cuda.stream(side) if side is not None else contextlib.nullcontext():
                ops.paged_decode(qkv[:nd], self.k_cache, self.v_cache, meta.d_block_tables,
                                 meta.d_seq_lens, Hq, Hkv, D, self.scale, self.window, self.sinks,
                                 split=meta.d_split, out=out[:nd], workspace=meta.d_workspace,
                                 max_ctx=meta.d_max_ctx, k_scale=self.k_scale, v_scale=self.v_scale,
                                 cascade=meta.d_cascade, split_dev=meta.d_split_dev)
        if meta.num_prefill_tokens:
            items = meta.p_items
            ops.paged_prefill(qkv[nd:], self.k_cache, self.v_cache, meta.p_block_tables,
                              meta.p_q_start, meta.p_q_len, meta.p_ctx_len, Hq, Hkv, D, self.scale,
                              self.window, self.sinks, items=items, out=out[nd:], k_scale=self.k_scale,
                              v_scale=self.v_scale)
        if side is not None:
            torch.cuda.current_stream(qkv.device).wait_stream(side)
        return out
```

### llmd_amd/models/llama.py

```python
from __future__ import annotations

from typing import Optional

import torch

from llmd_amd import ops
from llmd_amd.engine.attn_meta import AttnMeta
from llmd_amd.engine.config import ModelConfig
from llmd_amd.parallel.state import get_state

from .layers import ColumnLinear, LMHead, PagedAttention, RMSNorm, RowLinear, VocabEmbedding, wants_fp8_input


class LlamaMLP(torch.nn.Module):
    def __init__(self, cfg: ModelConfig, device):
        super().__init__()
        self.gate_up = ColumnLinear(cfg.hidden_size, 2 * cfg.intermediate_size, device=device)
        self.down = RowLinear(cfg.intermediate_size, cfg.hidden_size, device=device)

    def forward(self, x):
        return self.down(self.hidden(x))

    def hidden(self, x):
        gu = self.gate_up
        if (gu.lora is None and gu.bias is None and not wants_fp8_input(self.down) and x.dim() == 2
                and gu.weight.dtype == torch.bfloat16):
            v = ops.pgemm_silu_plan(x, gu.weight)
            if v is not None:
                return ops.pgemm_silu(x, gu.weight, variant=v)
            p = ops.mgemm_silu_plan(x, gu.weight)
            if p is not None:
                return ops.mgemm_silu(x, gu.weight, p)
        x0 = x[0] if isinstance(x, tuple) else x
        if (wants_fp8_input(self.down) and wants_fp8_input(gu) and gu.bias is None and x0.dim() == 2
                and ops._gpu(x0) and ops.pgemm8_silu_planned(x0.shape[0], gu.weight.shape[0], gu.weight.shape[1])):
            xq, xs = x if isinstance(x, tuple) else ops.quant_fp8_rows(x)
            if ops.pgemm_fp8_ok(xq, gu.weight):
                return ops.quant_fp8_rows(ops.pgemm_fp8(xq, xs, gu.weight, gu.weight_scale, epi=3))
        h = gu(x)
        if wants_fp8_input(self.down):
            return ops.gated_act_quant(h, ops.ACT_SILU)
        return ops.gated_act(h, ops.ACT_SILU)


def qkv_fused_plan(lin, x):
    if (not isinstance(x, torch.Tensor) or lin.bias is not None or lin.lora is not None
            or lin.weight.dtype != torch.bfloat16 or not (ops.MGEMM_NORM and ops._SKINNY)
            or lin.weight.shape[0] > 24576):
        return None
    if not (x.dim() == 2 and 33 <= x.shape[0] <= 128 and ops.mgemm_ok(x, lin.weight)):
        return None
    plan = ops.mgemm_choice(x.shape[0], lin.weight.shape[0], lin.weight.shape[1])
    return plan if plan is not None and plan[1] >= 2 and lin.weight.shape[1] // 64 >= 2 else None


def norm_fused_plan(lin, x):
    if (not isinstance(x, torch.Tensor) or lin.bias is not None or lin.lora is not None
            or lin.weight.dtype != torch.bfloat16 or (lin.reduce and get_state().tp_size > 1)):
        return None
    return ops.mgemm_norm_plan(x, lin.weight)


class LlamaDecoderLayer(torch.nn.Module):
    def __init__(self, cfg: ModelConfig, idx: int, cos_sin: torch.Tensor, device):
        super().__init__()
        d, D = cfg.hidden_size, cfg.head_dim
        Hq, Hkv = cfg.num_attention_heads, cfg.num_key_value_heads
        self.cfg = cfg
        self.input_layernorm = RMSNorm(d, cfg.rms_norm_eps, device)
        self.qkv = ColumnLinear(d, (Hq + 2 * Hkv) * D, bias=cfg.attention_bias, device=device)
        self.attn = PagedAttention(idx, Hq, Hkv, D, cos_sin, window=cfg.layer_window(idx),
                                   sinks=cfg.attention_sinks, device=device)
        self.o_proj = RowLinear(Hq * D, d, bias=cfg.attention_bias and cfg.model_type == "gpt_oss", device=device)
        self.post_attention_layernorm = RMSNorm(d, cfg.rms_norm_eps, device)
        self.mlp = self._make_mlp(cfg, idx, device)
        self.qk_norm = cfg.model_type in ("qwen3", "qwen3_moe")
        if self.qk_norm:
            self.q_norm = RMSNorm(D, cfg.rms_norm_eps, device)
            self.k_norm = RMSNorm(D, cfg.rms_norm_eps, device)

    def _make_mlp(self, cfg, idx, device):
        return LlamaMLP(cfg, device)

    def _apply_qk_norm(self, qkv):
        a = self.attn
        ops.qk_rms_norm(qkv, self.q_norm.weight, self.k_norm.weight, a.Hq, a.Hkv, self.q_norm.eps)

    def forward(self, x, residual, meta: AttnMeta):
        x, residual, _ = self.run(x, residual, meta)
        return x, residual

    def run(self, x, residual, meta: AttnMeta, normed: bool = False, next_norm: Optional[RMSNorm] = None):
        q_in = wants_fp8_input(self.qkv)
        if normed:
            pass
        elif residual is None:
            residual = x.clone()
            x = self.input_layernorm(x, quant=q_in)
        else:
            x, residual = self.input_layernorm(x, residual, quant=q_in)
        p = None if (self.qk_norm or q_in) else qkv_fused_plan(self.qkv, x)
        if p is not None:
            parts = ops.mgemm_partials(x, self.qkv.weight, p)
            a = self.attn(torch.empty(x.shape[0], self.qkv.weight.shape[0], dtype=x.dtype, device=x.device), meta,
                          parts=parts)
        else:
            qkv = self.qkv(x)
            if self.qk_norm:
                self._apply_qk_norm(qkv)
            a = self.attn(qkv, meta)
        q_mlp = isinstance(self.mlp, LlamaMLP) and wants_fp8_input(self.mlp.gate_up)
        p = None if q_mlp else norm_fused_plan(self.o_proj, a)
        if p is not None:
            pn = self.post_attention_layernorm
            x = ops.mgemm_add_rmsnorm(a, self.o_proj.weight, p, residual, pn.weight, pn.eps)
        else:
            x = self.o_proj(a)
            x, residual = self.post_attention_layernorm(x, residual, quant=q_mlp)
        if next_norm is not None and type(self.mlp) is LlamaMLP:
            h = self.mlp.hidden(x)
            p = norm_fused_plan(self.mlp.down, h)
            if p is not None:
                return ops.mgemm_add_rmsnorm(h, self.mlp.down.weight, p, residual, next_norm.weight,
                                             next_norm.eps), residual, True
            return self.mlp.down(h), residual, False
        return self.mlp(x), residual, False


class LlamaForCausalLM(torch.nn.Module):
    layer_cls = LlamaDecoderLayer

    def __init__(self, cfg: ModelConfig, device="cuda", max_pos: int = 32768):
        super().__init__()
        self.cfg = cfg
        rot = cfg.head_dim
        self.register_buffer("cos_sin", ops.rope_cos_sin(rot, max_pos, cfg.rope_theta, cfg.rope_scaling,
                                                         device=device), persistent=False)
        self.embed = VocabEmbedding(cfg.vocab_size, cfg.hidden_size, device)
        self.layers = torch.nn.ModuleList(
            [self.layer_cls(cfg, i, self.cos_sin, device) for i in range(cfg.num_hidden_layers)])
        self.norm = RMSNorm(cfg.hidden_size, cfg.rms_norm_eps, device)
        self.lm_head = LMHead(cfg.vocab_size, cfg.hidden_size, device,
                              tied=self.embed if cfg.tie_word_embeddings else None)

    def attention_layers(self):
        return [layer.attn for layer in self.layers]

    def weight_specs(self) -> list:
        cfg = self.cfg
        D, Hq, Hkv = cfg.head_dim, cfg.num_attention_heads, cfg.num_key_value_heads
        specs = [("model.embed_tokens.weight", self.embed.weight, "vocab", None),
                 ("model.norm.weight", self.norm.weight, "replicate", None)]
        if not cfg.tie_word_embeddings:
            specs.append(("lm_head.weight", self.lm_head.weight, "vocab", None))
        for i, layer in enumerate(self.layers):
            pre = f"model.layers.{i}."
            a = layer.attn
            q_rows, kv_rows = a.Hq * D, a.Hkv * D
            specs += [(pre + "input_layernorm.weight", layer.input_layernorm.weight, "replicate", None),
                      (pre + "post_attention_layernorm.weight", layer.post_attention_layernorm.weight,
                       "replicate", None),
                      (pre + "self_attn.o_proj.weight", layer.o_proj.weight, "row", None)]
            for nm, off, nh in (("q_proj", 0, Hq), ("k_proj", q_rows, Hkv), ("v_proj", q_rows + kv_rows, Hkv)):
                specs.append((pre + f"self_attn.{nm}.weight", layer.qkv.weight, "fused", (off, nh, D)))
                if layer.qkv.bias is not None:
                    specs.append((pre + f"self_attn.{nm}.bias", layer.qkv.bias, "fused", (off, nh, D)))
            if layer.o_proj.bias is not None:
                specs.append((pre + "self_attn.o_proj.bias", layer.o_proj.bias, "replicate", None))
            if layer.qk_norm:
                specs += [(pre + "self_attn.q_norm.weight", layer.q_norm.weight, "replicate", None),
                          (pre + "self_attn.k_norm.weight", layer.k_norm.weight, "replicate", None)]
            if a.sinks is not None:
                specs.append((pre + "self_attn.sinks", a.sinks, "col", None))
            specs += self._mlp_specs(pre, layer.mlp)
        return specs

    def _mlp_specs(self, pre: str, mlp) -> list:
        F_total = self.cfg.intermediate_size
        F_local = mlp.gate_up.weight.shape[0] // 2
        return [(pre + "mlp.gate_proj.weight", mlp.gate_up.weight, "fused", (0, F_total, 1)),
                (pre + "mlp.up_proj.weight", mlp.gate_up.weight, "fused", (F_local, F_total, 1)),
                (pre + "mlp.down_proj.weight", mlp.down.weight, "row", None)]

    @torch.no_grad()
    def forward(self, input_ids: torch.Tensor, meta: AttnMeta) -> torch.Tensor:
        x = self.embed(input_ids)
        residual = None
        normed = False
        n = len(self.layers)
        for i, layer in enumerate(self.layers):
            if not isinstance(layer, LlamaDecoderLayer) or type(layer).forward is not LlamaDecoderLayer.forward:
                x, residual = layer(x, residual, meta)
                normed = False
                continue
            nxt = self.layers[i + 1] if i + 1 < n else None
            if nxt is None:
                nn = self.norm
            elif (isinstance(nxt, LlamaDecoderLayer) and type(nxt).forward is LlamaDecoderLayer.forward
                  and not wants_fp8_input(nxt.qkv)):
                nn = nxt.input_layernorm
            else:
                nn = None
            x, residual, normed = layer.run(x, residual, meta, normed, nn)
        if normed:
            return x
        x, _ = self.norm(x, residual)
        return x

    @torch.no_grad()
    def compute_logits(self, h: torch.Tensor) -> torch.Tensor:
        return self.lm_head(h)


def kv_head_count(cfg: ModelConfig) -> int:
    return max(1, cfg.num_key_value_heads // get_state().tp_size)
```

### llmd_amd/ops/__init__.py

```python
from __future__ import annotations

import logging
import math
import os
from typing import Optional

import torch

from . import reference as ref

log = logging.getLogger("llmd.ops")

_C = None
_C_ERR: Exception | None = None


def native():
    global _C, _C_ERR
    if _C is not None:
        return _C
    import importlib

    debug = os.environ.get("LLMD_KERNEL_DEBUG", "0") == "1"
    name = "llmd_amd._C_debug" if debug else "llmd_amd._C"
# ... 935 lines not shown
                    best, best_t = (rb, ns2, occ), t
    return best


SKINNY_TUNED: dict[tuple[int, int, int], tuple[int, int, int]] = {}


def skinny_gemm(x: torch.Tensor, w: torch.Tensor, plan: Optional[tuple[int, int, int]] = None) -> torch.Tensor:
    M, K = x.shape
    N = w.shape[0]
    rb, ns, occ = plan or skinny_plan(M, N, K)
    y = torch.empty(M, N, dtype=x.dtype, device=x.device)
    part = torch.empty(ns * M * N if ns > 1 else 0, dtype=torch.float32, device=x.device)
    native().skinny_gemm(y, x, w, rb, ns, occ, part)
    return y


def skinny_ok(x: torch.Tensor, w: torch.Tensor) -> bool:
    M = x.shape[0] if x.dim() == 2 else -1
    return (_gpu(x) and 1 <= M <= SKINNY_MAX_M and x.shape[1] % 256 == 0 and x.dtype == torch.bfloat16
            and w.dtype == torch.bfloat16 and w.shape[0] % 4 == 0 and x.stride(-1) == 1 and x.stride(0) % 8 == 0
            and w.is_contiguous())


_DGEMM_MS = (1, 8, 16, 32, 48, 64)


def dgemm_choice(M: int, N: int, K: int) -> Optional[tuple[int, int, int]]:
    from .dgemm_table import DGEMM_TABLE

    for m in _DGEMM_MS:
        if m >= M:
            e = DGEMM_TABLE.get((m, N, K))
            return e[0] if e is not None else None
    return None


def mgemm(x: torch.Tensor, w: torch.Tensor, plan: tuple[int, int, int]) -> torch.Tensor:
    M, K = x.shape
    N = w.shape[0]
    wrb, ns, stages = plan
    y = torch.empty(M, N, dtype=x.dtype, device=x.device)
    part = torch.empty(ns * M * N if ns > 1 else 0, dtype=torch.float32, device=x.device)
    native().mgemm(y, x, w, wrb, ns, stages, part)
    return y


MGEMM_NORM = os.environ.get("LLMD_MGEMM_NORM", "1") == "1"


def mgemm_norm_plan(x: torch.Tensor, w: torch.Tensor) -> Optional[tuple[int, int, int]]:
    if not (MGEMM_NORM and _SKINNY and x.dim() == 2 and 33 <= x.shape[0] <= 128 and mgemm_ok(x, w)
            and w.shape[0] % 8 == 0 and w.shape[0] <= 8192 and w.shape[1] >= 128):
        return None
    plan = mgemm_choice(x.shape[0], w.shape[0], w.shape[1])
    if plan is None or plan[1] < 2:
        return None
    return plan


def mgemm_partials(x: torch.Tensor, w: torch.Tensor, plan: tuple[int, int, int]):
    M, N = x.shape[0], w.shape[0]
    part = torch.empty(plan[1] * M * N, dtype=torch.float32, device=x.device)
    ns = native().mgemm_partials(x, w, plan[0], plan[1], plan[2], part)
    return part, int(ns)


def reduce_rope_cache(part: torch.Tensor, nsplit: int, qkv: torch.Tensor, positions, cos_sin, Hq, Hkv, D, slots,
                      k_cache, v_cache, neox=True, k_scale=1.0, v_scale=1.0):
    native().reduce_rope_cache(part, nsplit, qkv, positions, cos_sin, Hq, Hkv, D, slots, k_cache, v_cache, neox,
                               k_scale, v_scale)


def mgemm_add_rmsnorm(x: torch.Tensor, w: torch.Tensor, plan: tuple[int, int, int], residual: torch.Tensor,
                      gamma: torch.Tensor, eps: float) -> torch.Tensor:
    M, N = x.shape[0], w.shape[0]
    wrb, ns, stages = plan
    out = torch.empty(M, N, dtype=x.dtype, device=x.device)
    part = torch.empty(ns * M * N, dtype=torch.float32, device=x.device)
    native().mgemm_add_rmsnorm(out, x, w, wrb, ns, stages, part, residual, gamma, eps)
    return out


MGEMM_SILU = os.environ.get("LLMD_MGEMM_SILU", "1") == "1"


def mgemm_silu_plan(x: torch.Tensor, w: torch.Tensor) -> Optional[tuple[int, int, int]]:
    if not (MGEMM_SILU and x.dim() == 2 and 33 <= x.shape[0] <= 256 and mgemm_ok(x, w) and w.shape[0] % 8 == 0):
        return None
    plan = mgemm_choice(x.shape[0], w.shape[0], w.shape[1])
    if plan is None or plan[1] != 1 or plan[0] not in (2, 4):
        return None
    if x.shape[0] > 128 and (plan[0], plan[2]) != (2, 3):
        return None
    return plan


def mgemm_silu(x: torch.Tensor, w: torch.Tensor, plan: tuple[int, int, int]) -> torch.Tensor:
    y = torch.empty(x.shape[0], w.shape[0] // 2, dtype=x.dtype, device=x.device)
    native().mgemm_silu(y, x, w, plan[0], plan[2])
    return y


def mgemm_fp8(xq: torch.Tensor, xs: torch.Tensor, wq: torch.Tensor, ws: torch.Tensor,
              plan: tuple[int, int, int]) -> torch.Tensor:
    M = xq.shape[0]
    N = wq.shape[0]
    wrb, ns, stages = plan
    y = torch.empty(M, N, dtype=torch.bfloat16, device=xq.device)
    part = torch.empty(ns * M * N if ns > 1 else 0, dtype=torch.float32, device=xq.device)
    native().mgemm_fp8(y, xq, xs, wq, ws, wrb, ns, stages, part)
    return y


def mgemm_fp8_choice(M: int, N: int, K: int) -> Optional[tuple[int, int, int]]:
    from .mgemm_fp8_table import MGEMM_FP8_TABLE

    if M < 33 or K % 128:
        return None
    for m in _MGEMM_MS:
        if m >= M:
            e = MGEMM_FP8_TABLE.get((m, N, K))
            return e[0] if e is not None else None
    return None


def mgemm_ok(x: torch.Tensor, w: torch.Tensor, max_m: int = 256) -> bool:
    M = x.shape[0] if x.dim() == 2 else -1
    return (_gpu(x) and 1 <= M <= max_m and x.shape[1] % 64 == 0 and x.dtype == torch.bfloat16
            and w.dtype == torch.bfloat16 and w.shape[0] % 4 == 0 and x.stride(-1) == 1 and x.stride(0) % 8 == 0
            and w.is_contiguous())


_MGEMM_MS = (64, 96, 128, 192, 256)


PGEMM_VARIANT = int(os.environ.get("LLMD_PGEMM_VARIANT", "0"))


def pgemm(x: torch.Tensor, w: torch.Tensor, epi: int = 0, out: Optional[torch.Tensor] = None,
          variant: Optional[int] = None, split_k: bool = True) -> torch.Tensor:
    M = x.shape[0]
    N = w.shape[0]
    if out is None:
        out = torch.empty(M, N // 2 if epi in (1, 3) else N, dtype=x.dtype, device=x.device)
    native().pgemm(out, x, w, epi, PGEMM_VARIANT if variant is None else variant, split_k)
    return out


def pgemm_silu(x: torch.Tensor, w: torch.Tensor, variant: int = 3, out: Optional[torch.Tensor] = None):
    return pgemm(x, w, epi=3, out=out, variant=variant, split_k=False)


def pgemm_pack_gate_up(w: torch.Tensor) -> torch.Tensor:
    F2, K = w.shape
    F = F2 // 2
    assert F % 128 == 0, F
    g = w[:F].view(F // 128, 128, K)
    u = w[F:].view(F // 128, 128, K)
    return torch.stack((g, u), 1).reshape(F2, K).contiguous()


def pgemm_ok(x: torch.Tensor, w: torch.Tensor) -> bool:
    return (x.dim() == 2 and x.dtype == torch.bfloat16 and w.dtype == torch.bfloat16 and x.is_cuda
            and w.shape[0] % 256 == 0 and w.shape[1] % 64 == 0 and x.stride(-1) == 1 and x.stride(0) % 8 == 0
            and w.is_contiguous())


def mgemm_choice(M: int, N: int, K: int) -> Optional[tuple[int, int, int]]:
    from .mgemm_table import MGEMM_TABLE

    for m in _MGEMM_MS:
        if m >= M:
            e = MGEMM_TABLE.get((m, N, K))
            return e[0] if e is not None else None
    return None


PGEMM_AUTO = os.environ.get("LLMD_PGEMM_AUTO", "table")
PGEMM_MIN_M = int(os.environ.get("LLMD_PGEMM_MIN_M", "256"))
_pgemm_pick: dict = {}


def _time_ms(fn, reps: int = 2) -> float:
    fn()
    st, en = torch.cuda.Event(enable_timing=True), torch.cuda.Event(enable_timing=True)
    st.record()
    for _ in range(reps):
        fn()
    en.record()
    en.synchronize()
    return st.elapsed_time(en) / reps


def pgemm_plan(M: int, N: int, K: int) -> Optional[tuple[int, bool]]:
    from .pgemm_table import PGEMM_TABLE

    e = PGEMM_TABLE.get(((M + 255) // 256, N, K))
    return None if e is None else e[0]


def pgemm_silu_plan(x: torch.Tensor, w: torch.Tensor) -> Optional[int]:
    if PGEMM_AUTO == "0" or x.shape[0] < PGEMM_MIN_M or not pgemm_ok(x, w) or (w.shape[0] // 2) % 128:
        return None
    from .pgemm_table import PGEMM_TABLE

    e = PGEMM_TABLE.get(("silu", (x.shape[0] + 255) // 256, w.shape[0], w.shape[1]))
    return None if e is None or e[0] is None else e[0][0]


def pgemm_wins(x: torch.Tensor, w: torch.Tensor) -> Optional[tuple[int, bool]]:
    M, (N, K) = x.shape[0], w.shape
    if PGEMM_AUTO != "measure":
        return pgemm_plan(M, N, K)
    key = ((M + 255) // 256, N, K)
    c = _pgemm_pick.get(key, False)
    if c is False:
        if torch.cuda.is_current_stream_capturing():
            return None
        y = torch.empty(M, N, dtype=x.dtype, device=x.device)
        t_pg = _time_ms(lambda: pgemm(x, w, out=y))
        t_bl = _time_ms(lambda: torch.nn.functional.linear(x, w))
        c = _pgemm_pick[key] = (PGEMM_VARIANT, True) if t_pg < 0.97 * t_bl else None
        msg = (f"prefill GEMM M~{M} N={N} K={K}: pgemm {t_pg:.3f} ms, hipBLASLt {t_bl:.3f} ms -> "
               f"{'pgemm' if c else 'hipBLASLt'}")
        log.debug(msg)
        if os.environ.get("LLMD_PGEMM_VERBOSE") == "1":
            import sys

            print(msg, file=sys.stderr, flush=True)
    return c


def linear(x: torch.Tensor, w: torch.Tensor, bias: Optional[torch.Tensor] = None) -> torch.Tensor:
    if PGEMM_AUTO != "0" and x.dim() == 2 and x.shape[0] >= PGEMM_MIN_M and pgemm_ok(x, w):
        plan = pgemm_wins(x, w)
        if plan is not None:
            y = pgemm(x, w, variant=plan[0], split_k=plan[1])
            return y if bias is None else y.add_(bias)
    if _SKINNY:
        M = x.shape[0] if x.dim() == 2 else 0
        if 33 <= M <= 256 and mgemm_ok(x, w):
            plan = mgemm_choice(M, w.shape[0], w.shape[1])
            if plan is not None:
                y = mgemm(x, w, plan)
                return y if bias is None else y.add_(bias)
        if skinny_ok(x, w):
            plan = dgemm_choice(M, w.shape[0], w.shape[1])
            if plan is not None:
                y = skinny_gemm(x, w, plan)
                return y if bias is None else y.add_(bias)
    return torch.nn.functional.linear(x, w, bias)


_SKINNY = os.environ.get("LLMD_SKINNY_GEMM", "1") == "1"
```

Before: 382.6 output tok/s (whole job).

## Fuse residual add and RoPE+KV-cache write into prefill GEMM epilogues

Adds two new epilogues to the variant-3 prefill bf16 GEMM. One adds the residual in place, used for o_proj and down_proj. The other applies NeoX RoPE and writes K/V straight into the paged KV cache, used for the QKV projection. The split-K reduce kernel gets matching epilogues. This removes the separate rope_cache and fused-add kernels and their extra round-trips of the QKV and residual tensors through HBM during prefill. In exchange, the epilogue carries more registers and extra loads, and the post-attention norm now runs as a separate norm call on the residual.

```diff
diff --git a/llmd_amd/csrc/ops/bindings.cpp b/llmd_amd/csrc/ops/bindings.cpp
--- a/llmd_amd/csrc/ops/bindings.cpp
+++ b/llmd_amd/csrc/ops/bindings.cpp
@@ -64,6 +64,10 @@
 int llmd_pgemm(const void*, int64_t, const void*, int64_t, void*, int64_t, int, int, int, int, int, void*,
                hipStream_t);
 int64_t llmd_pgemm_ws_bytes(int, int, int, int, int);
+int llmd_pgemm_add(const void*, int64_t, const void*, int64_t, void*, int64_t, int, int, int, int, void*, hipStream_t);
+int llmd_pgemm_rope_cache(const void*, int64_t, const void*, int64_t, void*, int64_t, int, int, int, int, void*,
+                          const int64_t*, const float*, int, int, const int64_t*, void*, void*, int64_t, int,
+                          hipStream_t);
 int llmd_pgemm_fp8(const void*, int64_t, const float*, const void*, int64_t, const float*, void*, int64_t, int, int,
                    int, int, void*, hipStream_t);
 int64_t llmd_pgemm_fp8_ws_bytes(int, int, int, int);
@@ -539,6 +543,61 @@
   TORCH_CHECK(rc == 0, "pgemm failed: ", rc);
 }
 
+void pgemm_add(torch::Tensor residual, torch::Tensor x, torch::Tensor w, int64_t variant, bool split_k) {
+  const c10::hip::OptionalHIPGuard device_guard(dev_of(residual));
+  CHECK_CUDA(x); CHECK_CUDA(residual); CHECK_BF16(x); CHECK_BF16(w); CHECK_BF16(residual);
+  CHECK_INNER(x); CHECK_INNER(w); CHECK_INNER(residual);
+  TORCH_CHECK(x.dim() == 2 && w.dim() == 2 && residual.dim() == 2, "pgemm_add: 2-D operands");
+  const int64_t M = x.size(0), K = x.size(1), N = w.size(0);
+  TORCH_CHECK(w.size(1) == K && K % 64 == 0 && N % 256 == 0, "pgemm_add: N % 256 == 0, K % 64 == 0");
+  TORCH_CHECK(residual.size(0) == M && residual.size(1) == N, "pgemm_add: residual shape");
+  TORCH_CHECK(variant == 3, "pgemm_add: variant 3 only");
+  TORCH_CHECK(x.stride(0) % 8 == 0 && w.stride(0) % 8 == 0 && residual.stride(0) % 8 == 0,
+              "pgemm_add: 16-B row alignment");
+  torch::Tensor ws;
+  const int64_t wsb = split_k ? llmd_pgemm_ws_bytes((int)M, (int)N, (int)K, 0, (int)variant) : 0;
+  if (wsb > 0) ws = torch::empty({wsb / 4}, x.options().dtype(torch::kFloat));
+  int rc = llmd_pgemm_add(x.data_ptr(), x.stride(0), w.data_ptr(), w.stride(0), residual.data_ptr(),
+                          residual.stride(0), (int)M, (int)N, (int)K, (int)variant, wsb > 0 ? ws.data_ptr() : nullptr,
+                          cur_stream());
+  TORCH_CHECK(rc == 0, "pgemm_add failed: ", rc);
+}
+
+void pgemm_rope_cache(torch::Tensor y, torch::Tensor x, torch::Tensor w, torch::Tensor positions,
+                      torch::Tensor cos_sin, int64_t Hq, int64_t Hkv, torch::Tensor slots, torch::Tensor k_cache,
+                      torch::Tensor v_cache, int64_t variant, bool split_k) {
+  const c10::hip::OptionalHIPGuard device_guard(dev_of(y));
+  CHECK_CUDA(x); CHECK_CUDA(y); CHECK_BF16(x); CHECK_BF16(w); CHECK_BF16(y); CHECK_INNER(x); CHECK_INNER(w); CHECK_INNER(y);
+  CHECK_DT(positions, at::kLong); CHECK_DT(slots, at::kLong); CHECK_DT(cos_sin, at::kFloat);
+  CHECK_CUDA(positions); CHECK_CUDA(slots); CHECK_CUDA(cos_sin); CHECK_CUDA(k_cache); CHECK_CUDA(v_cache);
+  TORCH_CHECK(x.dim() == 2 && w.dim() == 2 && y.dim() == 2, "pgemm_rope_cache: 2-D operands");
+  const int64_t M = x.size(0), K = x.size(1), N = w.size(0), D = 128;
+  TORCH_CHECK(w.size(1) == K && K % 64 == 0 && N % 256 == 0, "pgemm_rope_cache: N % 256 == 0, K % 64 == 0");
+  TORCH_CHECK(N == (Hq + 2 * Hkv) * D && y.size(0) == M && y.size(1) == N, "pgemm_rope_cache: heads of 128");
+  TORCH_CHECK(variant == 3, "pgemm_rope_cache: variant 3 only");
+  TORCH_CHECK(x.stride(0) % 8 == 0 && w.stride(0) % 8 == 0 && y.stride(0) % 8 == 0,
+              "pgemm_rope_cache: 16-B row alignment");
+  TORCH_CHECK(positions.numel() == M && slots.numel() == M && positions.is_contiguous() && slots.is_contiguous(),
+              "pgemm_rope_cache: positions / slots [M]");
+  TORCH_CHECK(cos_sin.dim() == 2 && cos_sin.is_contiguous() && cos_sin.size(1) == D,
+              "pgemm_rope_cache: cos_sin [pos, 128]");
+  TORCH_CHECK(k_cache.scalar_type() == at::kBFloat16 && v_cache.scalar_type() == at::kBFloat16,
+              "pgemm_rope_cache: bf16 caches");
+  TORCH_CHECK(k_cache.dim() == 4 && k_cache.size(1) == Hkv && k_cache.size(3) == D && k_cache.stride(3) == 1 &&
+              k_cache.stride(2) == D && k_cache.stride(1) == k_cache.size(2) * D && k_cache.stride(0) % 8 == 0 &&
+              v_cache.sizes() == k_cache.sizes() && v_cache.strides() == k_cache.strides(),
+              "pgemm_rope_cache: k/v cache layout");
+  torch::Tensor ws;
+  const int64_t wsb = split_k ? llmd_pgemm_ws_bytes((int)M, (int)N, (int)K, 0, (int)variant) : 0;
+  if (wsb > 0) ws = torch::empty({wsb / 4}, x.options().dtype(torch::kFloat));
+  int rc = llmd_pgemm_rope_cache(x.data_ptr(), x.stride(0), w.data_ptr(), w.stride(0), y.data_ptr(), y.stride(0),
+                                 (int)M, (int)N, (int)K, (int)variant, wsb > 0 ? ws.data_ptr() : nullptr,
+                                 positions.data_ptr<int64_t>(), cos_sin.data_ptr<float>(), (int)Hq, (int)Hkv,
+                                 slots.data_ptr<int64_t>(), k_cache.data_ptr(), v_cache.data_ptr(), k_cache.stride(0),
+                                 (int)k_cache.size(2), cur_stream());
+  TORCH_CHECK(rc == 0, "pgemm_rope_cache failed: ", rc);
+}
+
 void pgemm_fp8(torch::Tensor y, torch::Tensor xq, torch::Tensor xs, torch::Tensor wq, torch::Tensor ws, int64_t epi,
                bool split_k) {
   const c10::hip::OptionalHIPGuard device_guard(dev_of(y));
@@ -1265,6 +1324,9 @@
         "per-token x per-channel scales, optional fused SiLU-and-mul");
   m.def("pgemm", &pgemm, "prefill bf16 GEMM (256x256 LDS-DMA MFMA tiles), optional fused SiLU-and-mul",
         py::arg("y"), py::arg("x"), py::arg("w"), py::arg("epi"), py::arg("variant"), py::arg("split_k") = true);
+  m.def("pgemm_add", &pgemm_add, "prefill bf16 GEMM (variant 3) with the residual add in its epilogue, in place");
+  m.def("pgemm_rope_cache", &pgemm_rope_cache,
+        "prefill bf16 QKV GEMM (variant 3) with RoPE + the paged KV-cache write in its epilogue");
   m.def("mgemm_fp8", &mgemm_fp8);
   m.def("mgemm_lds", [](int64_t M, int64_t wrb, int64_t stages) { return llmd_mgemm_lds((int)M, (int)wrb, (int)stages); });
   m.def("lora_bgmv", &lora_bgmv);
diff --git a/llmd_amd/csrc/ops/pgemm.hip b/llmd_amd/csrc/ops/pgemm.hip
--- a/llmd_amd/csrc/ops/pgemm.hip
+++ b/llmd_amd/csrc/ops/pgemm.hip
@@ -13,7 +13,58 @@
 constexpr int LDS_BYTES = 2 * BUF;
 constexpr int GROUP_M = 8;
 
-enum { EPI_NONE = 0, EPI_SILU = 1, EPI_F32 = 2, EPI_SILU_STD = 3 };
+enum { EPI_NONE = 0, EPI_SILU = 1, EPI_F32 = 2, EPI_SILU_STD = 3, EPI_ADD = 4, EPI_ROPE = 5 };
+
+struct PgFuse {
+  uint16_t* res;
+  int64_t ldr;
+  const int64_t* pos;
+  const int64_t* slots;
+  const float* cos_sin;
+  uint16_t* kc;
+  uint16_t* vc;
+  int64_t block_stride;
+  int bs, Hq, Hkv;
+};
+
+__device__ __forceinline__ float partner8(float v) {
+  return __int_as_float(__builtin_amdgcn_update_dpp(0, __float_as_int(v), 0x128 , 0xf, 0xf, false));
+}
+__device__ __forceinline__ u32x4_t rope_chunk(const u32x4_t own, const u32x4_t partner, const f32x4_t cs0,
+                                              const f32x4_t cs1, bool low) {
+  float a[8], b[8], o[8];
+  unpack8(own, a);
+  unpack8(partner, b);
+#pragma unroll
+  for (int j = 0; j < 8; ++j) {
+    const float mine = j < 4 ? cs0[j & 3] : cs1[j & 3];
+    const float other = partner8(mine);
+    const float co = low ? mine : other, si = low ? -other : mine;
+    o[j] = __builtin_fmaf(a[j], co, b[j] * si);
+  }
+  return pack8(o);
+}
+
+__device__ __forceinline__ u32x4_t rope_pair(const u32x4_t lo, u32x4_t& hi, const f32x4_t co0, const f32x4_t co1,
+                                             const f32x4_t si0, const f32x4_t si1) {
+  float a[8], b[8], oa[8], ob[8];
+  unpack8(lo, a);
+  unpack8(hi, b);
+#pragma unroll
+  for (int j = 0; j < 8; ++j) {
+    const float co = j < 4 ? co0[j & 3] : co1[j & 3];
+    const float si = j < 4 ? si0[j & 3] : si1[j & 3];
+    oa[j] = __builtin_fmaf(a[j], co, -(b[j] * si));
+    ob[j] = __builtin_fmaf(b[j], co, a[j] * si);
+  }
+  hi = pack8(ob);
+  return pack8(oa);
+}
+
+__device__ __forceinline__ int64_t slot_offset(int64_t slot, int64_t block_stride, int bs) {
+  const uint32_t s = (uint32_t)slot, blk = s / (uint32_t)bs, r = s - blk * (uint32_t)bs;
+  return slot < 0 ? -1 : (int64_t)blk * block_stride + r * 128;
+}
 
 __device__ __forceinline__ void dma16(const void* src, char* lds) {
   __builtin_amdgcn_global_load_lds((const void __attribute__((address_space(1)))*)src,
@@ -640,7 +691,8 @@
 __global__ __launch_bounds__(NT6, 1) void pgemm6_kernel(const uint16_t* __restrict__ A, int64_t lda,
                                                         const uint16_t* __restrict__ W, int64_t ldw,
                                                         uint16_t* __restrict__ C, int64_t ldc, int M, int N, int K,
-                                                        int tile0, int nsplit, float* __restrict__ ws) {
+                                                        int tile0, int nsplit, float* __restrict__ ws,
+                                                        const PgFuse fz) {
   __shared__ __attribute__((aligned(1024))) char lds[2 * BUF6];
   const int tiles_m = (M + BM - 1) / BM, tiles_n = N / BN;
   const int b = xcd_remap(blockIdx.x, gridDim.x);
@@ -772,10 +824,52 @@
       }
     return;
   }
+  const int ec = lane & 15, er = lane >> 4;
+  const int pc = lane & 7, pr = lane >> 3;
+  const int mw = m0 + wr * 128;
+  [[maybe_unused]] u32x4_t rres[32];
+  [[maybe_unused]] int rpos[2];
+  [[maybe_unused]] int64_t roff[2];
+  [[maybe_unused]] f32x4_t rcs[2][4][4];
+  const int head = (n0 >> 7) + wc;
+  const bool rot_head = head < fz.Hq + fz.Hkv;
+  auto rope_pos = [&](int it) {
+    return __shfl(rpos[it >> 3], ((it & 7) << 3) + pr);
+  };
+  auto rope_load = [&](int bt) {
+#pragma unroll
+    for (int i = 0; i < 4; ++i) {
+      const float* p = fz.cos_sin + (int64_t)rope_pos(4 * bt + i) * 128 + pc * 8;
+      rcs[bt % 2][i][0] = *reinterpret_cast<const f32x4_t*>(p);
+      rcs[bt % 2][i][1] = *reinterpret_cast<const f32x4_t*>(p + 4);
+      rcs[bt % 2][i][2] = *reinterpret_cast<const f32x4_t*>(p + 64);
+      rcs[bt % 2][i][3] = *reinterpret_cast<const f32x4_t*>(p + 68);
+    }
+  };
+  auto res_load = [&](int it) {
+    const int m = min(mw + it * 4 + er, M - 1);
+    rres[it] = *reinterpret_cast<const u32x4_t*>(fz.res + (int64_t)m * fz.ldr + n0 + wc * 128 + ec * 8);
+  };
+  if constexpr (EPI == EPI_ADD) {
+#pragma unroll
+    for (int it = 0; it < 16; ++it) res_load(it);
+  }
+  if constexpr (EPI == EPI_ROPE) {
+    const int r0 = mw + lane, r1 = r0 + 64;
+    const int64_t p0 = fz.pos[min(r0, M - 1)], p1 = fz.pos[min(r1, M - 1)];
+    const int64_t s0 = fz.slots[min(r0, M - 1)], s1 = fz.slots[min(r1, M - 1)];
+    rpos[0] = (int)p0;
+    rpos[1] = (int)p1;
+    roff[0] = r0 < M ? slot_offset(s0, fz.block_stride, fz.bs) : -1;
+    roff[1] = r1 < M ? slot_offset(s1, fz.block_stride, fz.bs) : -1;
+    __builtin_amdgcn_sched_barrier(0);
+    rope_load(0);
+    rope_load(1);
+  }
   __syncthreads();
   char* img = lds + w * 32768;
 #pragma unroll
-  for (int i = 0; i < 8; ++i)
+  for (int i = 0; i < 8; ++i) {
 #pragma unroll
     for (int j = 0; j < 8; ++j) {
       const int row = 16 * i + fr, col = 16 * j + 4 * fq;
@@ -785,6 +879,8 @@
       p[1] = (uint32_t)f2bf(v[2]) | ((uint32_t)f2bf(v[3]) << 16);
       *reinterpret_cast<u32x2_t*>(img + row * 256 + (((col >> 3) ^ (row & 15)) * 16) + (col & 7) * 2) = p;
     }
+    if constexpr (EPI == EPI_ADD || EPI == EPI_ROPE) __builtin_amdgcn_sched_barrier(0);
+  }
   __syncthreads();
   if constexpr (EPI == EPI_NONE) {
 #pragma unroll 4
@@ -793,6 +889,55 @@
       const int m = m0 + wr * 128 + row;
       const u32x4_t v = *reinterpret_cast<const u32x4_t*>(img + row * 256 + ((c ^ (row & 15)) * 16));
       if (m < M) *reinterpret_cast<u32x4_t*>(C + (int64_t)m * ldc + n0 + wc * 128 + c * 8) = v;
+    }
+  } else if constexpr (EPI == EPI_ADD) {
+#pragma unroll
+    for (int it = 0; it < 32; ++it) {
+      if (it < 16) res_load(it + 16);
+      const int row = it * 4 + er, m = mw + row;
+      float a[8], r[8];
+      unpack8(*reinterpret_cast<const u32x4_t*>(img + row * 256 + ((ec ^ (row & 15)) * 16)), a);
+      unpack8(rres[it], r);
+#pragma unroll
+      for (int e = 0; e < 8; ++e) a[e] += r[e];
+      if (m < M) *reinterpret_cast<u32x4_t*>(fz.res + (int64_t)m * fz.ldr + n0 + wc * 128 + ec * 8) = pack8(a);
+      if (it % 4 == 3) __builtin_amdgcn_sched_barrier(0);
+    }
+  } else if constexpr (EPI == EPI_ROPE) {
+    auto cache_off = [&](int it) {
+      const int src = ((it & 7) << 3) + pr;
+      const uint32_t lo = __shfl((uint32_t)roff[it >> 3], src);
+      const uint32_t hi = __shfl((uint32_t)((uint64_t)roff[it >> 3] >> 32), src);
+      return (int64_t)(((uint64_t)hi << 32) | lo);
+    };
+    const int64_t kvh = (int64_t)(head - fz.Hq - (rot_head ? 0 : fz.Hkv)) * fz.bs * 128;
+    uint16_t* const cache = rot_head ? fz.kc : fz.vc;
+#pragma unroll
+    for (int bt = 0; bt < 4; ++bt) {
+#pragma unroll
+      for (int i = 0; i < 4; ++i) {
+        const int it = 4 * bt + i;
+        const int row = it * 8 + pr, m = mw + row;
+        u32x4_t lo = *reinterpret_cast<const u32x4_t*>(img + row * 256 + ((pc ^ (row & 15)) * 16));
+        u32x4_t hi = *reinterpret_cast<const u32x4_t*>(img + row * 256 + (((pc + 8) ^ (row & 15)) * 16));
+        if (rot_head)
+          lo = rope_pair(lo, hi, rcs[bt % 2][i][0], rcs[bt % 2][i][1], rcs[bt % 2][i][2], rcs[bt % 2][i][3]);
+        if (head < fz.Hq) {
+          uint16_t* dst = C + (int64_t)m * ldc + n0 + wc * 128 + pc * 8;
+          if (m < M) {
+            *reinterpret_cast<u32x4_t*>(dst) = lo;
+            *reinterpret_cast<u32x4_t*>(dst + 64) = hi;
+          }
+        } else {
+          const int64_t off = cache_off(it);
+          if (off >= 0) {
+            *reinterpret_cast<u32x4_t*>(cache + off + kvh + pc * 8) = lo;
+            *reinterpret_cast<u32x4_t*>(cache + off + kvh + 64 + pc * 8) = hi;
+          }
+        }
+      }
+      if (bt + 2 < 4) rope_load(bt + 2);
+      __builtin_amdgcn_sched_barrier(0);
     }
   } else {
     const char* gimg = lds + (wr * 2) * 32768;
@@ -1000,15 +1145,29 @@
   asm volatile("s_waitcnt vmcnt(0) lgkmcnt(0)" ::: "memory");
 }
 
+template <int EPI>
 __global__ __launch_bounds__(256) void pgemm_splitk_reduce(const float* __restrict__ ws, int nsplit, int tail,
                                                            int tile0, uint16_t* __restrict__ C, int64_t ldc, int M,
-                                                           int N) {
+                                                           int N, const PgFuse fz) {
   const int t = blockIdx.x / (BM / 8), rblk = blockIdx.x % (BM / 8);
   int tm, tn;
   tile_mn(tile0 + t, (M + BM - 1) / BM, N / BN, tm, tn);
   const int row = rblk * 8 + (threadIdx.x >> 5), col = (threadIdx.x & 31) * 8;
   const int m = tm * BM + row;
   if (m >= M) return;
+  [[maybe_unused]] u32x4_t res;
+  [[maybe_unused]] f32x4_t cs0 = {0.f, 0.f, 0.f, 0.f}, cs1 = {0.f, 0.f, 0.f, 0.f};
+  [[maybe_unused]] int64_t coff = -1;
+  const int head = (tn * BN + col) >> 7, ec = threadIdx.x & 15;
+  if constexpr (EPI == EPI_ADD) res = *reinterpret_cast<const u32x4_t*>(fz.res + (int64_t)m * fz.ldr + tn * BN + col);
+  if constexpr (EPI == EPI_ROPE) {
+    if (head < fz.Hq + fz.Hkv) {
+      const float* p = fz.cos_sin + fz.pos[m] * 128 + ec * 8;
+      cs0 = *reinterpret_cast<const f32x4_t*>(p);
+      cs1 = *reinterpret_cast<const f32x4_t*>(p + 4);
+    }
+    if (head >= fz.Hq) coff = slot_offset(fz.slots[m], fz.block_stride, fz.bs);
+  }
   float f[8] = {0, 0, 0, 0, 0, 0, 0, 0};
   for (int s = 0; s < nsplit; ++s) {
     const float* p = ws + ((int64_t)s * tail + t) * (BM * BN) + row * BN + col;
@@ -1019,7 +1178,29 @@
       f[4 + e] += b[e];
     }
   }
-  *reinterpret_cast<u32x4_t*>(C + (int64_t)m * ldc + tn * BN + col) = pack8(f);
+  const u32x4_t v = pack8(f);
+  if constexpr (EPI == EPI_ADD) {
+    float a[8], r[8];
+    unpack8(v, a);
+    unpack8(res, r);
+#pragma unroll
+    for (int e = 0; e < 8; ++e) a[e] += r[e];
+    *reinterpret_cast<u32x4_t*>(fz.res + (int64_t)m * fz.ldr + tn * BN + col) = pack8(a);
+  } else if constexpr (EPI == EPI_ROPE) {
+    u32x4_t par;
+#pragma unroll
+    for (int e = 0; e < 4; ++e) par[e] = __float_as_uint(partner8(__uint_as_float(v[e])));
+    const u32x4_t o = rope_chunk(v, par, cs0, cs1, ec < 8);
+    if (head < fz.Hq) {
+      *reinterpret_cast<u32x4_t*>(C + (int64_t)m * ldc + tn * BN + col) = o;
+    } else if (coff >= 0) {
+      const int kvh = head - fz.Hq;
+      if (kvh < fz.Hkv) *reinterpret_cast<u32x4_t*>(fz.kc + coff + (int64_t)kvh * fz.bs * 128 + ec * 8) = o;
+      else *reinterpret_cast<u32x4_t*>(fz.vc + coff + (int64_t)(kvh - fz.Hkv) * fz.bs * 128 + ec * 8) = v;
+    }
+  } else {
+    *reinterpret_cast<u32x4_t*>(C + (int64_t)m * ldc + tn * BN + col) = v;
+  }
 }
 
 constexpr int PG_CUS = 256;
@@ -1048,11 +1229,12 @@
   return nsplit > 1 ? (int64_t)nsplit * tail * BM * BN * 4 : 0;
 }
 
-extern "C" int llmd_pgemm(const void* A, int64_t lda, const void* W, int64_t ldw, void* C, int64_t ldc, int M, int N,
-                          int K, int epi, int variant, void* ws, hipStream_t st) {
+static int pgemm_launch(const void* A, int64_t lda, const void* W, int64_t ldw, void* C, int64_t ldc, int M, int N,
+                        int K, int epi, int variant, void* ws, hipStream_t st, const PgFuse& fz) {
   if (M <= 0) return 0;
   if (N % BN || K % BK || lda % 8 || ldw % 8 || ldc % 8) return -1;
   if (epi == EPI_SILU_STD && (variant < 3 || variant > 6)) return -3;
+  if ((epi == EPI_ADD || epi == EPI_ROPE) && variant != 3) return -3;
   if ((int64_t)(M - 1) * lda + K > 0x7fffffffLL || (int64_t)(N - 1) * ldw + K > 0x7fffffffLL) return -2;
   const int ntiles = ((M + BM - 1) / BM) * (N / BN);
   if (variant == 6) {
@@ -1071,31 +1253,56 @@
       return -3;
     if (nsplit > 1) {
       hipLaunchKernelGGL((pgemm6_kernel<EPI_F32, 37, 0>), dim3(tail * nsplit), dim3(NT6), 0, st, a, lda, w, ldw, c, ldc,
-                         M, N, K, full, nsplit, (float*)ws);
-      hipLaunchKernelGGL(pgemm_splitk_reduce, dim3(tail * (BM / 8)), dim3(256), 0, st, (const float*)ws, nsplit,
-                         tail, full, c, ldc, M, N);
+                         M, N, K, full, nsplit, (float*)ws, PgFuse{});
+      hipLaunchKernelGGL(pgemm_splitk_reduce<EPI_NONE>, dim3(tail * (BM / 8)), dim3(256), 0, st, (const float*)ws, nsplit,
+                         tail, full, c, ldc, M, N, PgFuse{});
     }
     return (int)hipGetLastError();
   }
   if (variant >= 3 && variant <= 5) {
     if (((int64_t)(M - 1) * lda + K) * 2 > 0x7fffffffLL || ((int64_t)(N - 1) * ldw + K) * 2 > 0x7fffffffLL) return -2;
     int full = ntiles, tail = 0, nsplit = 1;
-    if (ws != nullptr) pgemm_plan(M, N, K, epi, full, tail, nsplit);
+    const bool fused = epi == EPI_ADD || epi == EPI_ROPE;
+    if (ws != nullptr) pgemm_plan(M, N, K, fused ? EPI_NONE : epi, full, tail, nsplit);
     const auto* a = (const uint16_t*)A;
     const auto* w = (const uint16_t*)W;
     auto* c = (uint16_t*)C;
+    if (fused) {
+      if (epi == EPI_ADD) {
+        if (full > 0)
+          hipLaunchKernelGGL((pgemm6_kernel<EPI_ADD, 37, 0>), dim3(full), dim3(NT6), 0, st, a, lda, w, ldw, c, ldc, M, N,
+                             K, 0, 1, nullptr, fz);
+      } else if (full > 0) {
+        hipLaunchKernelGGL((pgemm6_kernel<EPI_ROPE, 37, 0>), dim3(full), dim3(NT6), 0, st, a, lda, w, ldw, c, ldc, M, N,
+                           K, 0, 1, nullptr, fz);
+      }
+      if (nsplit > 1) {
+        hipLaunchKernelGGL((pgemm6_kernel<EPI_F32, 37, 0>), dim3(tail * nsplit), dim3(NT6), 0, st, a, lda, w, ldw, c, ldc,
+                           M, N, K, full, nsplit, (float*)ws, PgFuse{});
+        if (epi == EPI_ADD)
+          hipLaunchKernelGGL(pgemm_splitk_reduce<EPI_ADD>, dim3(tail * (BM / 8)), dim3(256), 0, st, (const float*)ws,
+                             nsplit, tail, full, c, ldc, M, N, fz);
+        else
+          hipLaunchKernelGGL(pgemm_splitk_reduce<EPI_ROPE>, dim3(tail * (BM / 8)), dim3(256), 0, st, (const float*)ws,
+                             nsplit, tail, full, c, ldc, M, N, fz);
+      }
+      return (int)hipGetLastError();
+    }
     auto launch = [&](auto k_silu, auto k_std, auto k_none, auto k_f32) {
       if (epi == EPI_SILU)
-        hipLaunchKernelGGL(k_silu, dim3(full), dim3(NT6), 0, st, a, lda, w, ldw, c, ldc, M, N, K, 0, 1, nullptr);
+        hipLaunchKernelGGL(k_silu, dim3(full), dim3(NT6), 0, st, a, lda, w, ldw, c, ldc, M, N, K, 0, 1, nullptr,
+                           PgFuse{});
       else if (epi == EPI_SILU_STD)
-        hipLaunchKernelGGL(k_std, dim3(full), dim3(NT6), 0, st, a, lda, w, ldw, c, ldc, M, N, K, 0, 1, nullptr);
+        hipLaunchKernelGGL(k_std, dim3(full), dim3(NT6), 0, st, a, lda, w, ldw, c, ldc, M, N, K, 0, 1, nullptr,
+                           PgFuse{});
       else if (full > 0)
-        hipLaunchKernelGGL(k_none, dim3(full), dim3(NT6), 0, st, a, lda, w, ldw, c, ldc, M, N, K, 0, 1, nullptr);
+        hipLaunchKernelGGL(k_none, dim3(full), dim3(NT6), 0, st, a, lda, w, ldw, c, ldc, M, N, K, 0, 1, nullptr,
+                           PgFuse{});
       if (nsplit > 1) {
         hipLaunchKernelGGL(k_f32, dim3(tail * nsplit), dim3(NT6), 0, st, a, lda, w, ldw, c, ldc, M, N, K, full,
-                           nsplit, (float*)ws);
-        hipLaunchKernelGGL(pgemm_splitk_reduce, dim3(tail * (BM / 8)), dim3(256), 0, st, (const float*)ws, nsplit,
-                           tail, full, c, ldc, M, N);
+                           nsplit, (float*)ws, PgFuse{});
+        hipLaunchKernelGGL(pgemm_splitk_reduce<EPI_NONE>, dim3(tail * (BM / 8)), dim3(256), 0, st, (const float*)ws, nsplit,
+                           tail, full, c, ldc, M, N, PgFuse{});
       }
     };
     if (variant == 3)
@@ -1124,8 +1331,8 @@
     if (nsplit > 1) {
       hipLaunchKernelGGL(pgemm5_kernel<EPI_F32>, dim3(tail * nsplit), dim3(NT5), 0, st, a, lda, w, ldw, c, ldc, M, N,
                          K, full, nsplit, (float*)ws);
-      hipLaunchKernelGGL(pgemm_splitk_reduce, dim3(tail * (BM / 8)), dim3(256), 0, st, (const float*)ws, nsplit,
-                         tail, full, c, ldc, M, N);
+      hipLaunchKernelGGL(pgemm_splitk_reduce<EPI_NONE>, dim3(tail * (BM / 8)), dim3(256), 0, st, (const float*)ws, nsplit,
+                         tail, full, c, ldc, M, N, PgFuse{});
     }
     return (int)hipGetLastError();
   }
@@ -1144,8 +1351,8 @@
     if (nsplit > 1) {
       hipLaunchKernelGGL(pgemm4_kernel<EPI_F32>, dim3(tail * nsplit), dim3(NT4), 0, st, a, lda, w, ldw, c, ldc, M, N,
                          K, full, nsplit, (float*)ws);
-      hipLaunchKernelGGL(pgemm_splitk_reduce, dim3(tail * (BM / 8)), dim3(256), 0, st, (const float*)ws, nsplit,
-                         tail, full, c, ldc, M, N);
+      hipLaunchKernelGGL(pgemm_splitk_reduce<EPI_NONE>, dim3(tail * (BM / 8)), dim3(256), 0, st, (const float*)ws, nsplit,
+                         tail, full, c, ldc, M, N, PgFuse{});
     }
     return (int)hipGetLastError();
   }
@@ -1163,8 +1370,41 @@
   if (nsplit > 1) {
     hipLaunchKernelGGL(pgemm_kernel<EPI_F32>, dim3(tail * nsplit), dim3(NT), 0, st, a, lda, w, ldw, c, ldc, M, N, K,
                        full, nsplit, (float*)ws);
-    hipLaunchKernelGGL(pgemm_splitk_reduce, dim3(tail * (BM / 8)), dim3(256), 0, st, (const float*)ws, nsplit, tail,
-                       full, c, ldc, M, N);
+    hipLaunchKernelGGL(pgemm_splitk_reduce<EPI_NONE>, dim3(tail * (BM / 8)), dim3(256), 0, st, (const float*)ws, nsplit, tail,
+                       full, c, ldc, M, N, PgFuse{});
   }
   return (int)hipGetLastError();
 }
+
+extern "C" int llmd_pgemm(const void* A, int64_t lda, const void* W, int64_t ldw, void* C, int64_t ldc, int M, int N,
+                          int K, int epi, int variant, void* ws, hipStream_t st) {
+  if (epi == EPI_ADD || epi == EPI_ROPE) return -3;
+  return pgemm_launch(A, lda, W, ldw, C, ldc, M, N, K, epi, variant, ws, st, PgFuse{});
+}
+
+extern "C" int llmd_pgemm_add(const void* A, int64_t lda, const void* W, int64_t ldw, void* residual, int64_t ldr,
+                              int M, int N, int K, int variant, void* ws, hipStream_t st) {
+  if (ldr % 8) return -1;
+  PgFuse fz{};
+  fz.res = (uint16_t*)residual;
+  fz.ldr = ldr;
+  return pgemm_launch(A, lda, W, ldw, residual, ldr, M, N, K, EPI_ADD, variant, ws, st, fz);
+}
+
+extern "C" int llmd_pgemm_rope_cache(const void* A, int64_t lda, const void* W, int64_t ldw, void* C, int64_t ldc,
+                                     int M, int N, int K, int variant, void* ws, const int64_t* positions,
+                                     const float* cos_sin, int Hq, int Hkv, const int64_t* slots, void* kc, void* vc,
+                                     int64_t block_stride, int bs, hipStream_t st) {
+  if (Hq < 0 || Hkv < 0 || N != (Hq + 2 * Hkv) * 128 || bs <= 0 || block_stride % 8) return -1;
+  PgFuse fz{};
+  fz.pos = positions;
+  fz.slots = slots;
+  fz.cos_sin = cos_sin;
+  fz.kc = (uint16_t*)kc;
+  fz.vc = (uint16_t*)vc;
+  fz.block_stride = block_stride;
+  fz.bs = bs;
+  fz.Hq = Hq;
+  fz.Hkv = Hkv;
+  return pgemm_launch(A, lda, W, ldw, C, ldc, M, N, K, EPI_ROPE, variant, ws, st, fz);
+}
diff --git a/llmd_amd/models/layers.py b/llmd_amd/models/layers.py
--- a/llmd_amd/models/layers.py
+++ b/llmd_amd/models/layers.py
@@ -228,12 +228,16 @@
         self.k_scale = 1.0
         self.v_scale = 1.0
 
-    def forward(self, qkv: torch.Tensor, meta: AttnMeta, parts=None) -> torch.Tensor:
+    def layer_meta(self, meta: AttnMeta) -> AttnMeta:
+        return meta.swa if self.window and meta.swa is not None else meta
+
+    def forward(self, qkv: torch.Tensor, meta: AttnMeta, parts=None, roped: bool = False) -> torch.Tensor:
         T = qkv.shape[0]
         Hq, Hkv, D = self.Hq, self.Hkv, self.D
-        if self.window and meta.swa is not None:
-            meta = meta.swa
-        if parts is not None:
+        meta = self.layer_meta(meta)
+        if roped:
+            pass
+        elif parts is not None:
             ops.reduce_rope_cache(parts[0], parts[1], qkv, meta.positions, self.cos_sin, Hq, Hkv, D,
                                   meta.slot_mapping, self.k_cache, self.v_cache, self.neox, self.k_scale,
                                   self.v_scale)
diff --git a/llmd_amd/models/llama.py b/llmd_amd/models/llama.py
--- a/llmd_amd/models/llama.py
+++ b/llmd_amd/models/llama.py
@@ -61,6 +61,22 @@
     return ops.mgemm_norm_plan(x, lin.weight)
 
 
+def add_fused_plan(lin, x):
+    if (not isinstance(x, torch.Tensor) or lin.bias is not None or lin.lora is not None
+            or lin.weight.dtype != torch.bfloat16 or get_state().tp_size > 1):
+        return None
+    return ops.pgemm_fuse_plan(x, lin.weight, "add")
+
+
+def rope_fused_plan(lin, attn, x):
+    if (not isinstance(x, torch.Tensor) or lin.bias is not None or lin.lora is not None
+            or lin.weight.dtype != torch.bfloat16 or attn.k_cache is None
+            or lin.weight.shape[0] != (attn.Hq + 2 * attn.Hkv) * attn.D
+            or not ops.pgemm_rope_cache_ok(attn.D, attn.cos_sin.shape[1], attn.neox, attn.k_cache)):
+        return None
+    return ops.pgemm_fuse_plan(x, lin.weight, "rope")
+
+
 class LlamaDecoderLayer(torch.nn.Module):
     def __init__(self, cfg: ModelConfig, idx: int, cos_sin: torch.Tensor, device):
         super().__init__()
@@ -105,15 +121,27 @@
             a = self.attn(torch.empty(x.shape[0], self.qkv.weight.shape[0], dtype=x.dtype, device=x.device), meta,
                           parts=parts)
         else:
-            qkv = self.qkv(x)
-            if self.qk_norm:
-                self._apply_qk_norm(qkv)
-            a = self.attn(qkv, meta)
+            sk = None if (self.qk_norm or q_in) else rope_fused_plan(self.qkv, self.attn, x)
+            if sk is not None:
+                at = self.attn
+                m = at.layer_meta(meta)
+                qkv = ops.pgemm_rope_cache(x, self.qkv.weight, m.positions, at.cos_sin, at.Hq, at.Hkv, at.D,
+                                           m.slot_mapping, at.k_cache, at.v_cache, at.neox, 3, sk)
+                a = at(qkv, meta, roped=True)
+            else:
+                qkv = self.qkv(x)
+                if self.qk_norm:
+                    self._apply_qk_norm(qkv)
+                a = self.attn(qkv, meta)
         q_mlp = isinstance(self.mlp, LlamaMLP) and wants_fp8_input(self.mlp.gate_up)
         p = None if q_mlp else norm_fused_plan(self.o_proj, a)
+        sk = None if (q_mlp or p is not None) else add_fused_plan(self.o_proj, a)
         if p is not None:
             pn = self.post_attention_layernorm
             x = ops.mgemm_add_rmsnorm(a, self.o_proj.weight, p, residual, pn.weight, pn.eps)
+        elif sk is not None:
+            ops.pgemm_add(a, self.o_proj.weight, residual, 3, sk)
+            x = self.post_attention_layernorm(residual)
         else:
             x = self.o_proj(a)
             x, residual = self.post_attention_layernorm(x, residual, quant=q_mlp)
@@ -123,6 +151,10 @@
             if p is not None:
                 return ops.mgemm_add_rmsnorm(h, self.mlp.down.weight, p, residual, next_norm.weight,
                                              next_norm.eps), residual, True
+            sk = add_fused_plan(self.mlp.down, h)
+            if sk is not None:
+                ops.pgemm_add(h, self.mlp.down.weight, residual, 3, sk)
+                return next_norm(residual), residual, True
             return self.mlp.down(h), residual, False
         return self.mlp(x), residual, False
 
diff --git a/llmd_amd/ops/__init__.py b/llmd_amd/ops/__init__.py
--- a/llmd_amd/ops/__init__.py
+++ b/llmd_amd/ops/__init__.py
@@ -1111,6 +1111,48 @@
     return pgemm(x, w, epi=3, out=out, variant=variant, split_k=False)
 
 
+_PGEMM_FUSE_ENV = os.environ.get("LLMD_PGEMM_FUSE", "1")
+PGEMM_FUSE = _PGEMM_FUSE_ENV != "0"
+PGEMM_FUSE_KINDS = (_PGEMM_FUSE_ENV,) if _PGEMM_FUSE_ENV in ("add", "rope") else ("add", "rope")
+
+
+def pgemm_add(x: torch.Tensor, w: torch.Tensor, residual: torch.Tensor, variant: int = 3,
+              split_k: bool = True) -> torch.Tensor:
+    if not _gpu(x):
+        y = torch.nn.functional.linear(x, w)
+        residual.copy_((y.float() + residual.float()).to(residual.dtype))
+        return residual
+    native().pgemm_add(residual, x, w, variant, split_k)
+    return residual
+
+
+def pgemm_rope_cache_ok(D: int, rot: int, neox: bool, k_cache: torch.Tensor) -> bool:
+    return D == 128 and rot == D and bool(neox) and k_cache.dtype == torch.bfloat16
+
+
+def pgemm_rope_cache(x: torch.Tensor, w: torch.Tensor, positions, cos_sin, Hq: int, Hkv: int, D: int,
+                     slot_mapping, k_cache, v_cache, neox: bool = True, variant: int = 3,
+                     split_k: bool = True) -> torch.Tensor:
+    if (not _gpu(x) or not pgemm_rope_cache_ok(D, cos_sin.shape[1], neox, k_cache)
+            or w.shape[0] != (Hq + 2 * Hkv) * D):
+        qkv = pgemm(x, w, variant=variant, split_k=split_k) if _gpu(x) else torch.nn.functional.linear(x, w)
+        rope_cache(qkv, positions, cos_sin, Hq, Hkv, D, slot_mapping, k_cache, v_cache, neox)
+        return qkv
+    qkv = torch.empty(x.shape[0], w.shape[0], dtype=x.dtype, device=x.device)
+    native().pgemm_rope_cache(qkv, x, w, positions, cos_sin, Hq, Hkv, slot_mapping, k_cache, v_cache, variant,
+                              split_k)
+    return qkv
+
+
+def pgemm_fuse_plan(x, w: torch.Tensor, kind: str) -> Optional[bool]:
+    if not (PGEMM_FUSE and kind in PGEMM_FUSE_KINDS and PGEMM_AUTO == "table" and isinstance(x, torch.Tensor)
+            and x.dim() == 2
+            and x.shape[0] >= PGEMM_MIN_M and pgemm_ok(x, w)):
+        return None
+    plan = pgemm_plan(x.shape[0], w.shape[0], w.shape[1])
+    return plan[1] if plan is not None and plan[0] == 3 else None
+
+
 def pgemm_pack_gate_up(w: torch.Tensor) -> torch.Tensor:
     F2, K = w.shape
     F = F2 // 2
```

Result: no change. 383.8 output tok/s (whole job) (median of 6 runs) (+0.3%).
